# THUDM/GRAND-plus

Measured on AMD Instinct MI355X. Metric: propagation-matrix rows/sec (whole node), higher is better.
Workload: dtype f64

## Files before the change

grand_plus_amd/csrc/gfpush.hip:

```cpp
#include "gfpush_kernels.hpp"
#include "gfpush_sketch.hpp"
#ifndef GP_DIAG
#include "gfpush_dense.hpp"
#endif
#include "gfpush_plan.hpp"
#include "grandplus.h"

#include <dlfcn.h>
#include <sys/prctl.h>
#include <rccl/rccl.h>

#include <algorithm>
#include <atomic>
#include <cmath>
#include <cstdarg>
#include <cstdio>
#include <cstdlib>
#include <cstring>
#include <new>
#include <string>
#include <chrono>
#include <thread>
#include <type_traits>
#include <vector>
// ... 381 lines not shown

struct CallArgs {
    const int32_t* d_seeds; int64_t n_seeds; const double* coef; int n_coef; double rmax; int K;
    int32_t* d_row; int32_t* d_col; double* d_val; int32_t* d_filled; hipStream_t s;
};

struct CallShape : Shape {
    u64* timing_counters = nullptr;
    CallShape(const Shape& s, u64* tc = nullptr) : Shape(s), timing_counters(tc) {}
};

using Kernel = void (*)(KParams);
template <int... BLOCKS, class F> Kernel kernel_for(int block, F f) {
    Kernel k = nullptr;
    (void)(... || (block == BLOCKS && ((k = f(std::integral_constant<int, BLOCKS>())), true)));
    return k;
}

int resident_blocks(Kernel k, int block, int lds_bytes, int* out) {
    HIP_TRY(hipFuncSetAttribute(reinterpret_cast<const void*>(k), hipFuncAttributeMaxDynamicSharedMemorySize, lds_bytes));
    int nb = 0;
    HIP_TRY(hipOccupancyMaxActiveBlocksPerMultiprocessor(&nb, reinterpret_cast<const void*>(k), block, lds_bytes));
    *out = std::max(nb, 1);
    return GP_OK;
}
int launch_kernel(Kernel k, int block, const KParams& kp, int n_wg, int lds_bytes, hipStream_t s) {
    HIP_TRY(hipFuncSetAttribute(reinterpret_cast<const void*>(k), hipFuncAttributeMaxDynamicSharedMemorySize, lds_bytes));
    void* args[] = {const_cast<KParams*>(&kp)};
    (void)hipLaunchKernel(reinterpret_cast<const void*>(k), dim3(n_wg), dim3(block), args, lds_bytes, s);
    HIP_TRY(hipGetLastError());
    return GP_OK;
}

void use_slabs(KParams& kp, const Slabs& sl) {
    kp.push = sl.push; kp.push_cap = sl.push_cap;
    kp.bt = sl.bt; kp.bt_cap = sl.bt_cap;
    kp.resg = sl.resg; kp.resg_cap = sl.resg_cap;
    kp.log_key = sl.log_key; kp.log_val = sl.log_val; kp.log_cap = sl.log_cap;
    kp.log_pu = sl.log_pu; kp.arch = sl.arch; kp.arch_cap = sl.arch_cap;
    kp.cand = sl.cand; kp.cand_cap = sl.cand_cap;
    kp.bucket = sl.bucket; kp.bucket_cap = sl.bucket_cap;
}

void use_csr(KParams& kp, const gp_graph* g, bool acsr, bool general) {
    if (acsr) {
        kp.indices = g->d_acsr; kp.nnz = (int)(g->n_units << 5);
        kp.deg_shift = g->a_shift; kp.node_mask = g->a_mask; kp.deg_sat = g->a_sat;
        kp.node_pos = g->d_node_pos; kp.unit_info = g->d_unit_info; kp.sk_hub_units = g->a_sat > 32u ? 1u : 0u;
    } else {
        kp.indices = g->d_indices; kp.nnz = (int)g->nnz;
        kp.deg_shift = g->deg_shift; kp.node_mask = g->node_mask; kp.deg_sat = g->deg_sat;
    }
    kp.gk_acsr = acsr && general ? 1u : 0u;
}

int plan_status(Status st, const std::string& err) {
    return st == kOk ? GP_OK : fail(st == kNoMem ? GP_ERR_NOMEM : GP_ERR_INVALID_ARG, "%s", err.c_str());
}

#ifndef GP_DIAG
constexpr bool kDiagBuild = false;
Kernel sketch_kernel(int block) { return kernel_for<512, 1024, 768>(block, [](auto b) -> Kernel { return gfpush_sk_kernel<decltype(b)::value>; }); }

int plan_sketch(gp_graph* g, const CallArgs& a, const CallShape& shape, SketchPlan& p)
{
    sketch_wanted(kConsts, g->opt, g->est, shape, g->n_nodes, a.n_seeds, a.coef, a.n_coef, a.rmax, a.K, p);
    if (p.use) {
        int rc = ensure_acsr(g, a.s);
        if (rc) return rc;
        if (g->acsr_state != 1) p.use = false;
    }
    if (!p.use) return GP_OK;
    std::string err;
    int rc = plan_status(sketch_geometry(kConsts, g->opt, shape, a.K, p, err), err);
    if (rc || !p.use) return rc;
    int per_cu = 1;
    rc = resident_blocks(sketch_kernel(p.block), p.block, p.lds + g->opt.lds_pad, &per_cu);
    if (rc) return rc;
    p.wg = cap_workgroups(g->num_cus * per_cu, g->opt.max_workgroups, a.n_seeds);
    return GP_OK;
}

int launch_sketch(const gp_graph* g, KParams& kp, const CallArgs& a, const SketchPlan& sk, const u32* order)
{
    const Workspace& w = g->ws;
    use_slabs(kp, w.skl);
    kp.row_map = order; kp.n_rows_dev = nullptr; kp.queue_counter = kQueue;
    kp.retry_list = w.retry_list; kp.retry_counter = kRetryRows;
    kp.sk_lg_mu = sk.lg_mu; kp.sk_lg_mr = sk.lg_mr; kp.sk_cx = sk.cx;
    kp.sk_target = (u32)(g->opt.sk_target > 0 ? g->opt.sk_target : 4 * a.K);
    kp.sk_direct_max = g->opt.sk_direct_max > 0 ? (u32)g->opt.sk_direct_max : 0xFFFFFFFFu;
    kp.sk_rscale = 2147483648.0 / std::max(1.0, sk.coef_sum);
    {
        float t = (float)(a.rmax * 2147483648.0 * (1.0 - 1.0 / 1024.0));
        while ((double)t > a.rmax * 2147483648.0 * (1.0 - 1.0 / 1024.0)) t = std::nextafterf(t, 0.0f);
        kp.sk_thr_f = t;
    }
    use_csr(kp, g, true, false);
    return launch_kernel(sketch_kernel(sk.block), sk.block, kp, sk.wg, sk.lds + g->opt.lds_pad, a.s);
}
#else
constexpr bool kDiagBuild = true;
int plan_sketch(gp_graph*, const CallArgs&, const CallShape&, SketchPlan&) { return GP_OK; }
int launch_sketch(const gp_graph*, KParams&, const CallArgs&, const SketchPlan&, const u32*) { return GP_OK; }
#endif

Kernel general_kernel(int block) { return kernel_for<256, 512, 768, 1024>(block, [](auto b) -> Kernel { return gfpush_kernel<decltype(b)::value>; }); }
Kernel retry_kernel(int block) { return kernel_for<256, 512, 768, 1024>(block, [](auto b) -> Kernel { return gfpush_retry_kernel<decltype(b)::value>; }); }

int plan_general(gp_graph* g, const CallArgs& a, const CallShape& shape, SketchPlan& sk, GeneralPlan& p)
{
    CallInputs in;
    in.n_nodes = g->n_nodes; in.nnz = g->nnz; in.num_cus = g->num_cus;
    in.n_coef = a.n_coef; in.rmax = a.rmax; in.K = a.K; in.n_seeds = a.n_seeds;
    Occupancy occ;
    for (;;) {
        size_t free_b = 0, total_b = 0;
        const bool have_free = hipMemGetInfo(&free_b, &total_b) == hipSuccess;
        if (!have_free) (void)hipGetLastError();
        in.budget = workspace_budget(g->opt.workspace_mb, have_free, free_b, g->ws.bytes);
        Held held = g->ws.held();
        bool realloc = false; int need = 0; std::string err;
        Status st;
        while ((st = plan_general(kConsts, in, g->opt, shape, occ, sk, p, g->est, held, &realloc, &need, err)) == kNeedOccupancy) {
            int rc = resident_blocks(general_kernel(p.block_threads), p.block_threads, p.lds_bytes + g->opt.lds_pad, &occ.general[need]);
            if (rc) return rc;
        }
        if (st) return plan_status(st, err);
        if (!realloc) return GP_OK;
        int rc = allocate_workspace(g, held);
        if (rc == GP_ERR_NOMEM && sk.use && !shape.insists_on_sketch()) {
            sk.use = false; g_last_error.clear();
            continue;
        }
        return rc;
    }
}

KParams call_params(const gp_graph* g, const CallArgs& a, const GeneralPlan& gk, u64* counters)
{
    KParams kp;
    std::memset(&kp, 0, sizeof kp);
    kp.indptr = g->d_indptr; kp.indices = g->d_indices; kp.n_nodes = (int)g->n_nodes; kp.nnz = (int)g->nnz;
    kp.deg_shift = g->deg_shift; kp.node_mask = g->node_mask; kp.deg_sat = g->deg_sat;
    kp.seeds = a.d_seeds; kp.n_seeds = a.n_seeds;
    kp.coef = g->d_coef; kp.n_coef = a.n_coef; kp.rmax = a.rmax; kp.K = a.K;
    kp.out_row = a.d_row; kp.out_col = a.d_col; kp.out_val = a.d_val; kp.out_filled = a.d_filled;
    kp.counters = counters;
    kp.lds_slots = gk.lds_slots;
    kp.force_global = g->opt.force_global;
    kp.prune = prune_allowed(g->opt, a.coef, a.n_coef) ? 1 : 0;
    kp.diag_flags = g->opt.diag_flags;
    kp.rows_distinct = g->rows_distinct && g->opt.seedrow ? 1u : 0u;
    kp.solo = (g->opt.solo_levels ? 1u : 0u) | (g->opt.sk_seed_merge ? 2u : 0u);
    kp.direct = direct_tables(g->opt, g->n_nodes, gk) ? 1 : 0;
    return kp;
}

struct GeneralPass { const u32* rows; int n_rows; int queue; u32* overflow; int n_overflow; int overflow_queue; const u32* order; };

int launch_general(const gp_graph* g, KParams& kp, const GeneralPlan& gk, bool gk_acsr, const GeneralPass& pass, hipStream_t s)
{
    const Workspace& w = g->ws;
    const bool two_tier = w.big.n_wg > 0;
    use_csr(kp, g, gk_acsr, true);
    use_slabs(kp, w.est);
    kp.row_map = pass.rows ? pass.rows : pass.order; kp.n_rows_dev = pass.rows ? kp.counters + pass.n_rows : nullptr; kp.queue_counter = pass.queue;
    kp.retry_list = two_tier ? pass.overflow : nullptr; kp.retry_counter = pass.n_overflow;
    const Kernel k = pass.rows ? retry_kernel(gk.block_threads) : general_kernel(gk.block_threads);
    int rc = launch_kernel(k, gk.block_threads, kp, gk.n_wg, gk.lds_bytes + g->opt.lds_pad, s);
    if (rc || !two_tier) return rc;
    use_slabs(kp, w.big);
    kp.row_map = pass.overflow; kp.n_rows_dev = kp.counters + pass.n_overflow; kp.queue_counter = pass.overflow_queue;
    kp.retry_list = nullptr;
    return launch_kernel(retry_kernel(gk.block_threads), gk.block_threads, kp, w.big.n_wg, gk.lds_bytes + g->opt.lds_pad, s);
}

int enqueue_row_order(gp_graph* g, const CallArgs& a, bool acsr, hipStream_t s)
{
    const Workspace& w = g->ws;
    HIP_TRY(hipMemsetAsync(w.order_hist, 0, sizeof(uint32_t) * 64, s));
    const int shift = acsr ? g->a_shift : g->deg_shift;
    const u32 sat = acsr ? g->a_sat : g->deg_sat;
    const unsigned cost_wgs = (unsigned)std::min<int64_t>((a.n_seeds + 15) / 16, 4096), order_wgs = (unsigned)std::min<int64_t>((a.n_seeds + 255) / 256, 1024);
    hipLaunchKernelGGL(row_cost_kernel, dim3(cost_wgs), dim3(256), 0, s, a.d_seeds, (long long)a.n_seeds, (int)g->n_nodes, g->d_indptr,
                       acsr ? g->d_acsr : g->d_indices, acsr ? g->d_node_pos : (const u32*)nullptr, shift, sat, a.rmax, w.cost_cls, w.order_hist);
    hipLaunchKernelGGL(row_order_kernel, dim3(order_wgs), dim3(256), 0, s, w.cost_cls, (long long)a.n_seeds, w.order_hist, w.order_hist + 32, w.order);
    HIP_TRY(hipGetLastError());
    g->last_order_rows = a.n_seeds; g->last_order_sat = sat; g->last_order_shift = shift;
    return GP_OK;
}

int begin_call_state(gp_graph* g, const CallArgs& a, u64* counters, bool timing)
{
    const hipStream_t s = a.s;
    if (a.n_coef > g->coef_cap) {
        if (g->d_coef) (void)hipFree(g->d_coef);
        g->d_coef = nullptr; g->coef_cap = 0;
        HIP_TRY(hipMalloc(&g->d_coef, sizeof(double) * (size_t)a.n_coef));
        g->coef_cap = a.n_coef;
    }
    HIP_TRY(hipMemcpyAsync(g->d_coef, a.coef, sizeof(double) * (size_t)a.n_coef, hipMemcpyHostToDevice, s));
    if (timing || g->reset_pending) {
        HIP_TRY(hipMemsetAsync(counters, 0, sizeof(u64) * kNumCounters, s));
        if (!timing) { g->reset_pending = false; g->rows_total = 0; }
    } else {
        HIP_TRY(hipMemsetAsync(counters, 0, sizeof(u64) * (kSkSlabFails + 1), s));
        if (g->est.recipe_changed)
            HIP_TRY(hipMemsetAsync(counters + kMaxLevelEdges, 0, sizeof(u64) * 2, s));
    }
    g->est.recipe_changed = false;
    return GP_OK;
}

#ifndef GP_DIAG
static_assert(sizeof(DenseCtl) <= (size_t)kDenseCtlBytes, "DensePlan reserves kDenseCtlBytes for the dense kernel's control block");
Kernel dense_kernel(int block, bool staged) {
    return staged ? kernel_for<256, 512, 1024>(block, [](auto b) -> Kernel { return gfpush_dense_kernel<decltype(b)::value, true>; })
                  : kernel_for<256, 512, 1024>(block, [](auto b) -> Kernel { return gfpush_dense_kernel<decltype(b)::value, false>; });
}
bool dense_takes(const gp_graph* g, const CallArgs& a) {
    return dense_wanted(g->opt, g->n_nodes, g->nnz, a.n_coef, a.rmax, a.K, g->opt.lds_pad);
}

int enqueue_dense(gp_graph* g, const CallArgs& a, u64* counters, bool timing)
{
    const hipStream_t s = a.s;
    DensePlan dn = dense_plan(g->opt, g->n_nodes, g->nnz, a.K, g->opt.lds_pad);
    const Kernel k = dense_kernel(dn.block, dn.csr_lds);
    int per_cu = 1;
    int rc = resident_blocks(k, dn.block, dn.lds_bytes + g->opt.lds_pad, &per_cu);
    if (rc) return rc;
    dn = dense_plan(g->opt, g->n_nodes, g->nnz, a.K, g->opt.lds_pad, g->num_cus, per_cu, a.n_seeds);
    rc = ensure_packed(g, s);
    if (rc) return rc;
    rc = begin_call_state(g, a, counters, timing);
    if (rc) return rc;
    KParams kp = call_params(g, a, GeneralPlan(), counters);
    kp.direct = 0; kp.queue_counter = kQueue; kp.retry_counter = kRetryRows;
    kp.dn_hist = dn.off_hist; kp.dn_cur = dn.off_cur; kp.dn_next = dn.off_next; kp.dn_reserve = dn.off_reserve; kp.dn_marks = dn.off_marks;
    kp.dn_indptr = dn.off_indptr; kp.dn_indices = dn.off_indices; kp.dn_npad = (u32)dn.n_pad; kp.dn_csr_lds = dn.csr_lds ? 1u : 0u;
    HIP_TRY(hipEventRecord(g->ev0, s));
    g->last_order_rows = 0;
    if (a.n_seeds > 0) {
        rc = launch_kernel(k, dn.block, kp, dn.workgroups, dn.lds_bytes + g->opt.lds_pad, s);
        if (rc) return rc;
    }
    HIP_TRY(hipEventRecord(g->ev1, s));
    HIP_TRY(hipMemcpyAsync(g->h_counters, counters, sizeof(u64) * kNumCounters, hipMemcpyDeviceToHost, s));
    g->last_stream = s; g->est.last_call_rows = a.n_seeds; g->est.grown_for_call = false;
    g->est.last_kind = 3; g->est.last_sk_soft = false;
    if (timing) return GP_OK;
    g->launched = true;
    std::memset(&g->last, 0, sizeof g->last);
    g->rows_total += a.n_seeds;
    g->last.rows = g->rows_total;
    g->last.kernel = 3;
    g->last.workgroups = dn.workgroups; g->last.block_threads = dn.block; g->last.lds_bytes = dn.lds_bytes;
    return GP_OK;
}
#else
bool dense_takes(const gp_graph*, const CallArgs&) { return false; }
int enqueue_dense(gp_graph*, const CallArgs&, u64*, bool) { return GP_OK; }
#endif

int enqueue_call(gp_graph* g, const CallArgs& a, const CallShape& shape)
{
    const hipStream_t s = a.s;
    const bool timing = shape.timing_counters != nullptr;
    u64* const counters = timing ? shape.timing_counters : g->d_counters;
    if (g->launched && g->last_stream != s) HIP_TRY(hipStreamSynchronize(g->last_stream));
    if (!g->est.grown_for_call && g->est.rmax == a.rmax && g->est.n_coef == a.n_coef) {
        const hipError_t qs = hipStreamQuery(g->last_stream);
        if (qs == hipSuccess) grow_estimate(g);
        else if (qs != hipErrorNotReady) (void)hipGetLastError();
    }

    if (dense_takes(g, a)) return enqueue_dense(g, a, counters, timing);

    SketchPlan sk; GeneralPlan gk;
    int rc = plan_sketch(g, a, shape, sk);
    if (rc) return rc;
    rc = plan_general(g, a, shape, sk, gk);
    if (rc) return rc;
    rc = ensure_packed(g, s);
    if (rc) return rc;
    Workspace& w = g->ws;

    rc = begin_call_state(g, a, counters, timing);
    if (rc) return rc;
    if (w.dirty) {
        hipLaunchKernelGGL(init_tables_kernel, dim3(4096), dim3(256), 0, s, w.est.resg, (u64)w.est.n_wg * w.est.resg_cap);
        if (w.big.n_wg > 0)
            hipLaunchKernelGGL(init_tables_kernel, dim3(1024), dim3(256), 0, s, w.big.resg, (u64)w.big.n_wg * w.big.resg_cap);
        HIP_TRY(hipGetLastError());
        w.dirty = false;
    }

    KParams kp = call_params(g, a, gk, counters);
    bool gk_acsr = general_wants_acsr(kDiagBuild, g->opt, kp.direct != 0, g->n_nodes, a.n_seeds);
    if (gk_acsr) { rc = ensure_acsr(g, s); if (rc) return rc; gk_acsr = g->acsr_state == 1; }

    HIP_TRY(hipEventRecord(g->ev0, s));
    const u32* order = nullptr;
    g->last_order_rows = 0;
    if (g->opt.row_order && a.n_seeds > (sk.use ? sk.wg : gk.n_wg) && a.n_seeds <= w.retry_cap && a.n_seeds <= (int64_t)0xFFFFFFFFll) {
        rc = enqueue_row_order(g, a, sk.use || gk_acsr, s);
// ... 189 lines not shown
int gp_graph_create(const int32_t* indptr, int64_t n_nodes, const int32_t* indices, int64_t nnz,
                    int device, gp_graph** out)
{
    g_last_error.clear();
    if (!out) return fail(GP_ERR_NULL, "out is NULL");
    *out = nullptr;
    if (!indptr || (!indices && nnz > 0)) return fail(GP_ERR_NULL, "indptr/indices is NULL");
    if (n_nodes < 0 || nnz < 0 || n_nodes >= 2147483647ll || nnz >= 2147483647ll)
        return fail(GP_ERR_INVALID_CSR, "n_nodes=%lld nnz=%lld outside int32 CSR range", (long long)n_nodes, (long long)nnz);
    if (indptr[0] != 0) return fail(GP_ERR_INVALID_CSR, "indptr[0] = %d, expected 0", indptr[0]);
    for (int64_t i = 0; i < n_nodes; ++i)
        if (indptr[i + 1] < indptr[i]) return fail(GP_ERR_INVALID_CSR, "indptr decreases at node %lld", (long long)i);
    if (indptr[n_nodes] != nnz) return fail(GP_ERR_INVALID_CSR, "indptr[n] = %d but nnz = %lld", indptr[n_nodes], (long long)nnz);
    using clk = std::chrono::steady_clock;
    auto ms_since = [](clk::time_point t) { return std::chrono::duration<double, std::milli>(clk::now() - t).count(); };
    clk::time_point t0 = clk::now();
    const int ndev = gp_device_count();
    if (ndev <= 0) return fail(GP_ERR_NO_DEVICE, "no HIP device is visible (this library has no CPU path)");
    if (device < 0 || device >= ndev) return fail(GP_ERR_NO_DEVICE, "device %d outside [0, %d)", device, ndev);
    HIP_TRY(hipSetDevice(device));
    hipDeviceProp_t prop;
    HIP_TRY(hipGetDeviceProperties(&prop, device));
    g_create_ms[0] = ms_since(t0); t0 = clk::now();

    gp_graph* g = new (std::nothrow) gp_graph();
    if (!g) return fail(GP_ERR_NOMEM, "host allocation failed");
    g->device = device; g->n_nodes = n_nodes; g->nnz = nnz;
    g->num_cus = prop.multiProcessorCount;
    auto cleanup = [&](int status) { gp_graph_destroy(g); return status; };
    u32* d_flags = nullptr;
    {
        const size_t b_idx = (sizeof(int) * (size_t)(nnz + 1) + 255) & ~(size_t)255, b_ptr = (sizeof(int) * (size_t)(n_nodes + 1) + 255) & ~(size_t)255;
        if (hipMalloc(&g->d_csr_block, b_idx + b_ptr + 256) != hipSuccess)
            return cleanup(fail(GP_ERR_NOMEM, "hipMalloc of the CSR (%lld nodes, %lld nnz) failed", (long long)n_nodes, (long long)nnz));
        g->d_indices = (int*)g->d_csr_block; g->d_indptr = (int*)((char*)g->d_csr_block + b_idx); d_flags = (u32*)((char*)g->d_csr_block + b_idx + b_ptr);
    }
    if (hipStreamCreateWithFlags(&g->stream, hipStreamNonBlocking) != hipSuccess)
        return cleanup(fail(GP_ERR_HIP, "creating per-graph HIP objects failed"));
    g_create_ms[1] = ms_since(t0); t0 = clk::now();
    Stager stager;
    if (stager.copy(g->d_indptr, indptr, sizeof(int) * (size_t)(n_nodes + 1), g->stream) != GP_OK ||
        (nnz > 0 && stager.copy(g->d_indices, indices, sizeof(int) * (size_t)nnz, g->stream) != GP_OK) ||
        hipMemsetAsync(g->d_indices + nnz, 0xFF, sizeof(int), g->stream) != hipSuccess ||
        hipMemsetAsync(d_flags, 0, sizeof(u32) * 2, g->stream) != hipSuccess)
        return cleanup(fail(GP_ERR_HIP, "CSR upload failed"));
    g_create_ms[2] = ms_since(t0); t0 = clk::now();
    u32 h_flags[2] = {0u, 0u};
    if (n_nodes > 0) hipLaunchKernelGGL(csr_check_kernel, dim3(8192), dim3(256), 0, g->stream, g->d_indptr, g->d_indices, (long long)n_nodes, d_flags);
    if (hipGetLastError() != hipSuccess ||
        hipMemcpyAsync(h_flags, d_flags, sizeof h_flags, hipMemcpyDeviceToHost, g->stream) != hipSuccess ||
        hipStreamSynchronize(g->stream) != hipSuccess)
        return cleanup(fail(GP_ERR_HIP, "CSR validation on the device failed"));
    if (h_flags[0]) return cleanup(fail(GP_ERR_INVALID_CSR, "a column id is outside [0, %lld)", (long long)n_nodes));
    g->rows_distinct = h_flags[1] == 0;
    g_create_ms[3] = ms_since(t0); t0 = clk::now();
    if (hipMalloc(&g->d_counters, sizeof(u64) * kNumCounters) != hipSuccess ||
        hipHostMalloc(&g->h_counters, sizeof(u64) * kNumCounters) != hipSuccess ||
        hipEventCreate(&g->ev0) != hipSuccess || hipEventCreate(&g->ev1) != hipSuccess)
        return cleanup(fail(GP_ERR_HIP, "creating per-graph HIP objects failed"));
    g_create_ms[4] = ms_since(t0);
    *out = g;
    return GP_OK;
}

void gp_graph_destroy(gp_graph* g) {
    if (!g) return;
    if (g->multi) {
        for (size_t d = 0; d < g->comms.size(); ++d) if (g->comms[d]) (void)g_rccl.CommDestroy(g->comms[d]);
        for (size_t d = 0; d < g->part.size(); ++d) {
            if (!g->part[d]) continue;
            (void)hipSetDevice(g->devices[d]);
            if (d < g->m_slab.size() && g->m_slab[d]) (void)hipFree(g->m_slab[d]);
            if (d < g->m_gather.size() && g->m_gather[d]) (void)hipFree(g->m_gather[d]);
            if (d < g->m_seeds.size() && g->m_seeds[d]) (void)hipFree(g->m_seeds[d]);
            gp_graph_destroy(g->part[d]);
        }
        if (g->m_host) (void)hipHostFree(g->m_host);
        delete g;
        return;
    }
    (void)hipSetDevice(g->device);
    if (g->launched) (void)hipStreamSynchronize(g->last_stream);
    free_workspace(g->ws);
    if (g->d_csr_block) (void)hipFree(g->d_csr_block);
    else {
        if (g->d_indptr) (void)hipFree(g->d_indptr);
        if (g->d_indices) (void)hipFree(g->d_indices);
    }
    if (g->d_acsr) (void)hipFree(g->d_acsr);
    if (g->d_node_pos) (void)hipFree(g->d_node_pos);
    if (g->d_unit_info) (void)hipFree(g->d_unit_info);
    if (g->d_counters) (void)hipFree(g->d_counters);
    if (g->d_cal_counters) (void)hipFree(g->d_cal_counters);
    if (g->d_wg_log) (void)hipFree(g->d_wg_log);
    if (g->h_counters) (void)hipHostFree(g->h_counters);
    if (g->d_coef) (void)hipFree(g->d_coef);
    if (g->d_seeds) (void)hipFree(g->d_seeds);
    for (int i = 0; i < 2; ++i) if (g->h_slab[i]) (void)hipHostFree(g->h_slab[i]);
    if (g->ev0) (void)hipEventDestroy(g->ev0);
    if (g->ev1) (void)hipEventDestroy(g->ev1);
    if (g->stream) (void)hipStreamDestroy(g->stream);
    delete g;
}

int64_t gp_graph_num_nodes(const gp_graph* g) { return g ? g->n_nodes : -1; }
int64_t gp_graph_nnz(const gp_graph* g) { return g ? g->nnz : -1; }
int gp_graph_device(const gp_graph* g) { return g ? (g->multi ? g->devices[0] : g->device) : -1; }
int gp_graph_num_gpus(const gp_graph* g) { return g ? (g->multi ? g->n_parts : 1) : -1; }

int gp_set_option(gp_graph* g, const char* key, int64_t value) {
    if (!g || !key) return fail(GP_ERR_NULL, "null argument");
    const std::string k(key);
    if (g->multi) {
        if (k == "force_collective") { g->force_collective = value ? 1 : 0; return GP_OK; }
        if (k == "gather_host") {
            if (!value && g->shared_devices) return fail(GP_ERR_INVALID_ARG, "parts of this handle share a device: RCCL takes one rank per device, the gather stays on the host");
            g->gather_host = value ? 1 : 0; return GP_OK;
        }
        if (k == "min_rows_per_gpu") {
            if (value < 1) return fail(GP_ERR_INVALID_ARG, "min_rows_per_gpu must be >= 1");
            g->min_rows_per_gpu = value; return GP_OK;
        }
        for (gp_graph* q : g->part) if (q) { int rc = gp_set_option(q, key, value); if (rc) return rc; }
        return GP_OK;
    }
    if (k == "block_threads") {
        if (value != 256 && value != 512 && value != 768 && value != 1024) return fail(GP_ERR_INVALID_ARG, "block_threads must be 256, 512, 768 or 1024");
        g->opt.block_threads = (int)value;
    } else if (k == "lds_bytes") {
        if (value < 40 * 1024 || value > 160 * 1024) return fail(GP_ERR_INVALID_ARG, "lds_bytes must be in [40960, 163840]");
        g->opt.lds_bytes = (int)(value & ~15ll);
    } else if (k == "lds_pad") {
        if (value < 0 || value > 120 * 1024) return fail(GP_ERR_INVALID_ARG, "lds_pad must be in [0, 122880]");
        g->opt.lds_pad = (int)(value & ~15ll);
    } else if (k == "kernel") {
        if (value < 0 || value > 3) return fail(GP_ERR_INVALID_ARG, "kernel must be 0 (automatic), 1 (general), 2 (sketch) or 3 (dense)");
        g->opt.kernel = (int)value;
    } else if (k == "dn_block_threads") {
        if (value != 0 && value != 256 && value != 512 && value != 1024) return fail(GP_ERR_INVALID_ARG, "dn_block_threads must be 0, 256, 512 or 1024");
        g->opt.dn_block = (int)value;
    } else if (k == "dn_csr_lds") {
        g->opt.dn_csr_lds = value ? 1 : 0;
    } else if (k == "sk_block_threads") {
        if (value != 0 && value != 512 && value != 768 && value != 1024) return fail(GP_ERR_INVALID_ARG, "sk_block_threads must be 0, 512, 768 or 1024");
        g->opt.sk_block = (int)value;
    } else if (k == "sk_lg_mu" || k == "sk_lg_mr") {
        if (value != 0 && (value < 8 || value > 14)) return fail(GP_ERR_INVALID_ARG, "%s must be 0 or in [8, 14]", key);
        (k == "sk_lg_mu" ? g->opt.sk_lg_mu : g->opt.sk_lg_mr) = (int)value;
    } else if (k == "sk_direct_max") {
        if (value < 0 || value > (1 << 20)) return fail(GP_ERR_INVALID_ARG, "sk_direct_max must be in [0, 2^20]");
        g->opt.sk_direct_max = (int)value;
    } else if (k == "sk_seed_merge") {
        g->opt.sk_seed_merge = value ? 1 : 0;
    } else if (k == "row_order") {
        g->opt.row_order = value ? 1 : 0;
    } else if (k == "gk_acsr") {
        g->opt.gk_acsr = value ? 1 : 0;
    } else if (k == "sk_target") {
        if (value < 0 || value > 4096) return fail(GP_ERR_INVALID_ARG, "sk_target must be in [0, 4096]");
        g->opt.sk_target = (int)value;
    } else if (k == "measure_choice") {
        g->opt.measure_choice = value ? 1 : 0;
        if (!value) g->choices.clear();
    } else if (k == "verify_merge") {
        g->opt.verify_merge = value ? 1 : 0;
    } else if (k == "pretouch") {
        g->opt.pretouch = value ? 1 : 0;
    } else if (k == "max_workgroups") {
        if (value < 0 || value > 65535) return fail(GP_ERR_INVALID_ARG, "max_workgroups must be in [0, 65535]");
        g->opt.max_workgroups = (int)value;
    } else if (k == "workspace_mb") {
        if (value < 1) return fail(GP_ERR_INVALID_ARG, "workspace_mb must be >= 1");
        g->opt.workspace_mb = value;
    } else if (k == "est_level_edges") {
        if (value < 0) return fail(GP_ERR_INVALID_ARG, "est_level_edges must be >= 0");
        g->opt.est_level_edges = value;
    } else if (k == "force_global") {
        g->opt.force_global = value ? 1 : 0;
    } else if (k == "exact_stats") {
        g->opt.exact_stats = value ? 1 : 0;
    } else if (k == "direct_tables") {
        g->opt.direct_tables = value ? 1 : 0;
    } else if (k == "solo_levels") {
        g->opt.solo_levels = value ? 1 : 0;
    } else if (k == "seedrow") {
        g->opt.seedrow = value ? 1 : 0;
    } else if (k == "diag_flags") {
        g->opt.diag_flags = (int)value;
    } else if (k == "max_degree_bits") {
        if (g->packed) return fail(GP_ERR_INVALID_ARG, "max_degree_bits must be set before the first gfpush call");
        if (value < 0 || value > 31) return fail(GP_ERR_INVALID_ARG, "max_degree_bits must be in [0, 31]");
        g->opt.max_degree_bits = (int)value;
    } else {
        return fail(GP_ERR_INVALID_ARG, "unknown option '%s'", key);
    }
    if (k == "max_workgroups" || k == "workspace_mb" || k == "lds_pad" || k == "est_level_edges" || k.rfind("sk_", 0) == 0 || k.rfind("dn_", 0) == 0 ||
        k == "solo_levels" || k == "seedrow" || k == "direct_tables") g->choices.clear();
    return GP_OK;
}

int gp_gfpush_device(gp_graph* g, const int32_t* d_seeds, int64_t n_seeds,
                     const double* coef, int n_coef, double rmax, int K,
                     int32_t* d_row, int32_t* d_col, double* d_val, int32_t* d_filled, void* stream)
{
    g_last_error.clear();
    int rc = check_call_args(g, n_seeds, coef, n_coef, rmax, K);
    if (rc) return rc;
    if (g->multi) return fail(GP_ERR_INVALID_ARG, "gp_gfpush_device needs a single-GPU graph (device buffers live on one GPU); "
                                                  "a multi-GPU handle takes host buffers through gp_gfpush");
    if (n_seeds > 0 && (!d_seeds || !d_row || !d_col || !d_val)) return fail(GP_ERR_NULL, "a device buffer is NULL");
    HIP_TRY(hipSetDevice(g->device));
    const CallArgs a{d_seeds, n_seeds, coef, n_coef, rmax, K, d_row, d_col, d_val, d_filled, (hipStream_t)stream};
    const gp_graph::Choice* c = nullptr;
    rc = measured_choice(g, a, &c);
    if (rc) return rc;
    CallShape shape(Shape{g->opt.kernel, g->opt.block_threads, g->opt.lds_bytes, false});
    if (c) shape = CallShape(Shape{c->kernel, c->block_threads, c->lds_bytes, true});
    if (c) std::memcpy(g->last_cal_ms, c->ms, sizeof g->last_cal_ms);
    else std::memset(g->last_cal_ms, 0, sizeof g->last_cal_ms);
    return enqueue_call(g, a, shape);
}

int gp_reset_stats(gp_graph* g) {
    if (!g) return fail(GP_ERR_NULL, "graph handle is NULL");
    if (g->multi) { for (gp_graph* q : g->part) if (q) (void)gp_reset_stats(q); g->m_has_stats = false; return GP_OK; }
    g->reset_pending = true;
    return GP_OK;
}

int gp_get_stats(gp_graph* g, gp_stats* out) {
    if (!g) return fail(GP_ERR_NULL, "graph handle is NULL");
    if (g->multi) {
        if (out) { if (g->m_has_stats) *out = g->m_last; else std::memset(out, 0, sizeof *out); }
        if (g->m_has_stats && g->m_last.failed_rows)
            return fail(GP_ERR_OVERFLOW, "%lld row(s) hit a workspace bound", (long long)g->m_last.failed_rows);
        return GP_OK;
    }
    if (!g->launched) { if (out) std::memset(out, 0, sizeof *out); return GP_OK; }
    HIP_TRY(hipSetDevice(g->device));
    HIP_TRY(hipStreamSynchronize(g->last_stream));
    float ms = 0.f;
    HIP_TRY(hipEventElapsedTime(&ms, g->ev0, g->ev1));
    gp_stats& s = g->last;
    s.kernel_ms = ms;
    s.pushes = (int64_t)g->h_counters[kPushes];
    s.edges = (int64_t)g->h_counters[kEdges];
    s.filled = (int64_t)g->h_counters[kFilled];
    s.support = (int64_t)g->h_counters[kSupport];
    s.frontier = (int64_t)g->h_counters[kFrontier];
    s.lds_levels = (int64_t)g->h_counters[kLdsLevels];
    s.global_levels = (int64_t)g->h_counters[kGlobalLevels];
    s.failed_rows = (int64_t)g->h_counters[kFailedRows];
    s.degree_lookups = (int64_t)g->h_counters[kDegLookups];
    s.retried_rows = (int64_t)g->h_counters[kRetriedTotal];
    s.max_level_edges = (int64_t)g->h_counters[kMaxLevelEdges];
    s.max_log_records = (int64_t)g->h_counters[kMaxLogRecords];
    s.sketch_candidate_edges = (int64_t)g->h_counters[kSkCandEdges];
    s.sketch_second_sweeps = (int64_t)g->h_counters[kSkSweep2];
    for (int i = 0; i < 3; ++i) s.choice_ms[i] = g->last_cal_ms[i];
    grow_estimate(g);
    s.diag_ticks_scan = (int64_t)g->h_counters[kTicksScan];
    s.diag_ticks_expand = (int64_t)g->h_counters[kTicksExpand];
    s.diag_ticks_topk = (int64_t)g->h_counters[kTicksTopk];
    s.diag_ticks_total = (int64_t)g->h_counters[kTicksTotal];
    s.diag_ticks_scan_hbm = (int64_t)g->h_counters[kTicksScanHbm];
    s.diag_ticks_expand_hbm = (int64_t)g->h_counters[kTicksExpandHbm];
    for (int i = 0; i < 16; ++i) s.diag_sub[i] = (int64_t)g->h_counters[kDiag0 + i];
    if (out) *out = s;
    if (s.failed_rows) {
        g->ws.dirty = true;
        return fail(GP_ERR_OVERFLOW, "%lld row(s) hit a workspace bound or had an out-of-range seed", (long long)s.failed_rows);
    }
    return GP_OK;
}

int gp_gfpush(gp_graph* g, const int32_t* seeds, int64_t n_seeds,
              const double* coef, int n_coef, double rmax, int K,
              int32_t* row_idx, int32_t* col_idx, double* value)
{
    g_last_error.clear();
    int rc = check_call_args(g, n_seeds, coef, n_coef, rmax, K);
    if (rc) return rc;
    if (n_seeds == 0) return GP_OK;
    if (!seeds || !row_idx || !col_idx || !value) return fail(GP_ERR_NULL, "a host buffer is NULL");
    for (int64_t i = 0; i < n_seeds; ++i)
        if (seeds[i] < 0 || seeds[i] >= g->n_nodes)
            return fail(GP_ERR_INVALID_SEED, "node_idx[%lld] = %d outside [0, %lld)", (long long)i, seeds[i], (long long)g->n_nodes);
    if (g->multi) return gfpush_multi(g, seeds, n_seeds, coef, n_coef, rmax, K, row_idx, col_idx, value);
    HIP_TRY(hipSetDevice(g->device));
    if (n_seeds > g->seeds_cap) {
        if (g->d_seeds) (void)hipFree(g->d_seeds);
        g->d_seeds = nullptr; g->seeds_cap = 0;
        HIP_TRY(hipMalloc(&g->d_seeds, sizeof(int) * (size_t)n_seeds));
        g->seeds_cap = n_seeds;
    }
    const PackedSlab lay(n_seeds, K);
    const size_t need_bytes = lay.bytes;
    if (need_bytes > g->out_bytes) {
        for (int i = 0; i < 2; ++i) { if (g->h_slab[i]) (void)hipHostFree(g->h_slab[i]); g->h_slab[i] = nullptr; g->h_slab_clean[i] = false; }
        g->out_bytes = 0;
        for (int i = 0; i < 2; ++i) HIP_TRY(hipHostMalloc(&g->h_slab[i], need_bytes, hipHostMallocMapped | hipHostMallocCoherent));
        g->out_bytes = need_bytes;
    }
    const int cur = g->h_slab_next; g->h_slab_next ^= 1;
    char* hb = g->h_slab[cur];
    if (!g->h_slab_clean[cur]) std::memset(hb, 0xFF, g->out_bytes);
    g->h_slab_clean[cur] = false;
    char* idle = g->h_slab[cur ^ 1]; size_t idle_done = g->h_slab_clean[cur ^ 1] ? g->out_bytes : 0;
    double* d_val = nullptr; int* d_row = nullptr; int* d_col = nullptr; int* d_filled = nullptr;
    {
        void* dp = nullptr;
        HIP_TRY(hipHostGetDevicePointer(&dp, hb, 0));
        d_val = (double*)((char*)dp + lay.val); d_row = (int*)((char*)dp + lay.row); d_col = (int*)((char*)dp + lay.col); d_filled = (int*)((char*)dp + lay.filled);
    }
    hipStream_t s = g->stream;
    g->reset_pending = true;
    HIP_TRY(hipMemcpyAsync(g->d_seeds, seeds, sizeof(int) * (size_t)n_seeds, hipMemcpyHostToDevice, s));
    rc = gp_gfpush_device(g, g->d_seeds, n_seeds, coef, n_coef, rmax, K, d_row, d_col, d_val, d_filled, s);
    if (rc) return rc;
    MergeState merge;
    std::vector<unsigned char>& done = g->h_done;
    done.assign((size_t)n_seeds, 0);
    auto sweep = [&]() { merge_sweep(hb, lay, K, n_seeds, done.data(), merge, row_idx, col_idx, value); };
    struct Resetter {
        std::thread t;
        ~Resetter() { if (t.joinable()) t.join(); }
    } resetter;
    bool reset_inline = false;
    if (idle_done < g->out_bytes) {
        const size_t n_reset = g->out_bytes;
        try { resetter.t = std::thread([idle, n_reset]() { std::memset(idle, 0xFF, n_reset); }); }
        catch (...) { reset_inline = true; }
    }
    struct TimerSlack {
        long old = -1;
        TimerSlack() { old = prctl(PR_GET_TIMERSLACK, 0, 0, 0, 0); if (old > 0) (void)prctl(PR_SET_TIMERSLACK, 1000UL, 0, 0, 0); }
        ~TimerSlack() { if (old > 0) (void)prctl(PR_SET_TIMERSLACK, (unsigned long)old, 0, 0, 0); }
    } timer_slack;
    for (;;) {
        const hipError_t q = hipStreamQuery(s);
        if (q == hipSuccess) break;
        if (q != hipErrorNotReady) { (void)hipGetLastError(); break; }
        const int64_t before = merge.n_merged;
        sweep();
        if (merge.n_merged - before < 256) std::this_thread::sleep_for(std::chrono::microseconds(60));
    }
    if (resetter.t.joinable()) { resetter.t.join(); g->h_slab_clean[cur ^ 1] = true; }
    else if (reset_inline) { std::memset(idle, 0xFF, g->out_bytes); g->h_slab_clean[cur ^ 1] = true; }
    rc = gp_get_stats(g, nullptr);
    if (rc) return rc;
    for (int spin = 0; merge.n_merged != n_seeds && spin < 2000000; ++spin) sweep();
    if (merge.n_merged != n_seeds) return fail(GP_ERR_HIP, "%lld of %lld rows never arrived in host memory", (long long)(n_seeds - merge.n_merged), (long long)n_seeds);
    if (g->opt.verify_merge) {
        int64_t first_bad = -1;
        const int64_t bad = verify_merged(hb, lay, K, n_seeds, row_idx, col_idx, value, &first_bad);
        if (bad) return fail(GP_ERR_HIP, "verify_merge: %lld of %lld rows were merged before they had fully arrived (first: row %lld)",
                             (long long)bad, (long long)n_seeds, (long long)first_bad);
    }
    return GP_OK;
}

int gp_graph_create_multi_on(const int32_t* indptr, int64_t n_nodes, const int32_t* indices, int64_t nnz,
                             const int* devices, int n_parts, gp_graph** out)
{
    g_last_error.clear();
    if (!out) return fail(GP_ERR_NULL, "out is NULL");
    *out = nullptr;
    if (!devices || n_parts < 1) return fail(GP_ERR_INVALID_ARG, "gp_graph_create_multi_on needs at least one device");
    const int ndev = gp_device_count();
    if (ndev <= 0) return fail(GP_ERR_NO_DEVICE, "no HIP device is visible (this library has no CPU path)");
    bool repeated = false;
    for (int d = 0; d < n_parts; ++d) {
        if (devices[d] < 0 || devices[d] >= ndev) return fail(GP_ERR_NO_DEVICE, "device %d outside [0, %d)", devices[d], ndev);
        for (int e = 0; e < d; ++e) repeated |= devices[e] == devices[d];
    }
    gp_graph* first = nullptr;
    int rc = gp_graph_create(indptr, n_nodes, indices, nnz, devices[0], &first);
    if (rc) return rc;
    gp_graph* g = new (std::nothrow) gp_graph();
    if (!g) { gp_graph_destroy(first); return fail(GP_ERR_NOMEM, "host allocation failed"); }
    g->multi = true; g->n_parts = n_parts; g->n_nodes = n_nodes; g->nnz = nnz;
    g->part.assign(n_parts, nullptr); g->devices.assign(devices, devices + n_parts);
    g->part[0] = first;
    g->comms.assign(n_parts, nullptr);
    g->m_slab.assign(n_parts, nullptr); g->m_gather.assign(n_parts, nullptr); g->m_seeds.assign(n_parts, nullptr);
    g->shared_devices = repeated;
    if (repeated) g->gather_host = 1;
    *out = g;
    return GP_OK;
}

int gp_graph_create_multi(const int32_t* indptr, int64_t n_nodes, const int32_t* indices, int64_t nnz,
                          int n_gpus, gp_graph** out)
{
    g_last_error.clear();
    if (!out) return fail(GP_ERR_NULL, "out is NULL");
    *out = nullptr;
    const int ndev = gp_device_count();
    if (ndev <= 0) return fail(GP_ERR_NO_DEVICE, "no HIP device is visible (this library has no CPU path)");
    if (n_gpus < 0 || n_gpus > ndev) return fail(GP_ERR_NO_DEVICE, "n_gpus = %d but %d device(s) are visible", n_gpus, ndev);
    if (n_gpus == 0) n_gpus = ndev;
    std::vector<int> devs(n_gpus);
    for (int d = 0; d < n_gpus; ++d) devs[d] = d;
    return gp_graph_create_multi_on(indptr, n_nodes, indices, nnz, devs.data(), n_gpus, out);
}

}

namespace {

int replicate_part(gp_graph* g, int d) {
    gp_graph* src = g->part[0];
    HIP_TRY(hipSetDevice(src->device));
    int rc = ensure_packed(src, src->stream);
    if (rc) return rc;
    HIP_TRY(hipStreamSynchronize(src->stream));
    const int dev = g->devices[d];
    HIP_TRY(hipSetDevice(dev));
    hipDeviceProp_t prop;
    HIP_TRY(hipGetDeviceProperties(&prop, dev));
    gp_graph* q = new (std::nothrow) gp_graph();
    if (!q) return fail(GP_ERR_NOMEM, "host allocation failed");
    struct Guard { gp_graph* q; ~Guard() { if (q) gp_graph_destroy(q); } } guard{q};
    q->device = dev; q->n_nodes = src->n_nodes; q->nnz = src->nnz; q->num_cus = prop.multiProcessorCount;
    q->deg_shift = src->deg_shift; q->node_mask = src->node_mask; q->deg_sat = src->deg_sat;
    q->packed = true; q->opt.max_degree_bits = src->opt.max_degree_bits; q->rows_distinct = src->rows_distinct;
    q->opt.block_threads = src->opt.block_threads; q->opt.lds_bytes = src->opt.lds_bytes; q->opt.max_workgroups = src->opt.max_workgroups;
    q->opt.workspace_mb = src->opt.workspace_mb; q->opt.force_global = src->opt.force_global; q->opt.exact_stats = src->opt.exact_stats;
    q->opt.direct_tables = src->opt.direct_tables; q->opt.est_level_edges = src->opt.est_level_edges; q->opt.seedrow = src->opt.seedrow; q->opt.solo_levels = src->opt.solo_levels;
    q->opt.kernel = src->opt.kernel; q->opt.row_order = src->opt.row_order; q->opt.gk_acsr = src->opt.gk_acsr; q->opt.sk_seed_merge = src->opt.sk_seed_merge; q->opt.sk_block = src->opt.sk_block; q->opt.sk_lg_mu = src->opt.sk_lg_mu; q->opt.sk_lg_mr = src->opt.sk_lg_mr; q->opt.sk_target = src->opt.sk_target; q->opt.lds_pad = src->opt.lds_pad; q->opt.sk_direct_max = src->opt.sk_direct_max;
    const size_t b_ptr = sizeof(int) * (size_t)(q->n_nodes + 1), b_idx = sizeof(int) * (size_t)(q->nnz + 1);
    HIP_TRY(hipMalloc(&q->d_indptr, b_ptr));
    HIP_TRY(hipMalloc(&q->d_indices, b_idx));
    if (dev == src->device) {
        HIP_TRY(hipMemcpy(q->d_indptr, src->d_indptr, b_ptr, hipMemcpyDeviceToDevice));
        HIP_TRY(hipMemcpy(q->d_indices, src->d_indices, b_idx, hipMemcpyDeviceToDevice));
    } else {
        HIP_TRY(hipMemcpyPeer(q->d_indptr, dev, src->d_indptr, src->device, b_ptr));
        HIP_TRY(hipMemcpyPeer(q->d_indices, dev, src->d_indices, src->device, b_idx));
    }
    HIP_TRY(hipMalloc(&q->d_counters, sizeof(u64) * kNumCounters));
    HIP_TRY(hipHostMalloc(&q->h_counters, sizeof(u64) * kNumCounters));
    HIP_TRY(hipEventCreate(&q->ev0));
    HIP_TRY(hipEventCreate(&q->ev1));
    HIP_TRY(hipStreamCreateWithFlags(&q->stream, hipStreamNonBlocking));
    guard.q = nullptr;
    g->part[d] = q;
    return GP_OK;
}

int gfpush_multi(gp_graph* g, const int32_t* seeds, int64_t n_seeds, const double* coef, int n_coef, double rmax, int K,
                 int32_t* row_idx, int32_t* col_idx, double* value)
{
    const MultiPlan plan = plan_multi(n_seeds, K, g->n_parts, g->min_rows_per_gpu, g->force_collective != 0, g->gather_host != 0);
    const int G = plan.G, Gc = plan.Gc;
    if (plan.single) {
        int rc = gp_gfpush(g->part[0], seeds, n_seeds, coef, n_coef, rmax, K, row_idx, col_idx, value);
        gp_stats st; const int rc2 = gp_get_stats(g->part[0], &st);
        g->m_last = st; g->m_has_stats = true;
        return rc ? rc : rc2;
    }
    const bool collective = !g->gather_host;
    for (int d = 1; d < Gc; ++d)
        if (!g->part[d]) { int rc = replicate_part(g, d); if (rc) return rc; }
    if (collective && !g->comms_ready) {
        int rc = load_rccl();
        if (rc) return rc;
        RCCL_TRY(g_rccl.CommInitAll(g->comms.data(), g->n_parts, g->devices.data()));
        g->comms_ready = true;
    }
    const int64_t per = plan.per;
    const size_t stride = plan.stride;
    if (g->m_cap_stride.size() != (size_t)g->n_parts) { g->m_cap_stride.assign(g->n_parts, 0); g->m_cap_per.assign(g->n_parts, 0); }
    for (int d = 0; d < Gc; ++d) {
        if (g->m_slab[d] && g->m_cap_stride[d] >= stride && g->m_cap_per[d] >= per) continue;
        HIP_TRY(hipSetDevice(g->devices[d]));
        if (g->m_slab[d]) (void)hipFree(g->m_slab[d]);
        if (g->m_gather[d]) (void)hipFree(g->m_gather[d]);
        if (g->m_seeds[d]) (void)hipFree(g->m_seeds[d]);
        g->m_slab[d] = g->m_gather[d] = nullptr; g->m_seeds[d] = nullptr; g->m_cap_stride[d] = 0; g->m_cap_per[d] = 0;
        const size_t cap_s = std::max(stride, g->m_cap_stride[d]);
        const int64_t cap_p = std::max<int64_t>(std::max(per, g->m_cap_per[d]), 1);
        HIP_TRY(hipMalloc(&g->m_slab[d], cap_s));
        HIP_TRY(hipMalloc(&g->m_gather[d], cap_s * (size_t)g->n_parts));
        HIP_TRY(hipMalloc(&g->m_seeds[d], sizeof(int) * (size_t)cap_p));
        g->m_cap_stride[d] = cap_s; g->m_cap_per[d] = cap_p;
    }
    if (stride * (size_t)g->n_parts > g->m_host_bytes) {
        if (g->m_host) (void)hipHostFree(g->m_host);
        g->m_host = nullptr; g->m_host_bytes = 0;
        HIP_TRY(hipSetDevice(g->devices[0]));
        HIP_TRY(hipHostMalloc(&g->m_host, stride * (size_t)g->n_parts));
        g->m_host_bytes = stride * (size_t)g->n_parts;
    }
    const size_t cur_stride = stride;
    const int64_t cur_per = per;
    const PackedSlab lay(cur_per, K);

    std::vector<int> rcs(Gc, GP_OK);
    std::vector<std::string> errs(Gc);
    std::vector<std::thread> pool;
    auto work = [&](int d) {
        gp_graph* q = g->part[d];
        int64_t lo, n;
        plan_block(plan, d, n_seeds, &lo, &n);
        auto run = [&]() -> int {
            HIP_TRY(hipSetDevice(q->device));
            char* slab = g->m_slab[d];
            HIP_TRY(hipMemsetAsync(slab + lay.filled, 0, 4 * (size_t)cur_per, q->stream));
            if (n > 0) {
                HIP_TRY(hipMemcpyAsync(g->m_seeds[d], seeds + lo, sizeof(int) * (size_t)n, hipMemcpyHostToDevice, q->stream));
                q->reset_pending = true;
                int rc = gp_gfpush_device(q, g->m_seeds[d], n, coef, n_coef, rmax, K, (int*)(slab + lay.row),
                                          (int*)(slab + lay.col), (double*)(slab + lay.val), (int*)(slab + lay.filled), q->stream);
                if (rc) return rc;
            }
            if (!collective) HIP_TRY(hipMemcpyAsync(g->m_host + (size_t)d * cur_stride, slab, cur_stride, hipMemcpyDeviceToHost, q->stream));
            return GP_OK;
        };
        rcs[d] = run();
        if (rcs[d]) errs[d] = g_last_error;
    };
    for (int d = 1; d < Gc; ++d) pool.emplace_back(work, d);
    work(0);
    for (auto& th : pool) th.join();
    for (int d = 0; d < Gc; ++d) if (rcs[d]) { g_last_error = errs[d]; return rcs[d]; }

    if (collective) {
        RCCL_TRY(g_rccl.GroupStart());
        for (int d = 0; d < Gc; ++d)
            RCCL_TRY(g_rccl.AllGather(g->m_slab[d], g->m_gather[d], cur_stride, ncclUint8, g->comms[d], g->part[d]->stream));
        RCCL_TRY(g_rccl.GroupEnd());
        HIP_TRY(hipSetDevice(g->devices[0]));
        HIP_TRY(hipMemcpyAsync(g->m_host, g->m_gather[0], cur_stride * (size_t)Gc, hipMemcpyDeviceToHost, g->part[0]->stream));
    }
    gp_stats sum; std::memset(&sum, 0, sizeof sum);
    int status = GP_OK;
    for (int d = 0; d < Gc; ++d) {
        gp_graph* q = g->part[d];
        HIP_TRY(hipSetDevice(q->device));
        HIP_TRY(hipStreamSynchronize(q->stream));
        int64_t lo_d, n_d;
        plan_block(plan, d, n_seeds, &lo_d, &n_d);
        if (!q->launched || n_d == 0) continue;
        gp_stats st; const int rc = gp_get_stats(q, &st);
        if (rc && !status) status = rc;
        sum.rows += st.rows; sum.pushes += st.pushes; sum.edges += st.edges; sum.filled += st.filled; sum.support += st.support;
        sum.frontier += st.frontier; sum.lds_levels += st.lds_levels; sum.global_levels += st.global_levels;
        sum.failed_rows += st.failed_rows; sum.degree_lookups += st.degree_lookups; sum.retried_rows += st.retried_rows;
        sum.kernel_ms = std::max(sum.kernel_ms, st.kernel_ms); sum.workgroups += st.workgroups;
        sum.block_threads = st.block_threads; sum.lds_bytes = st.lds_bytes; sum.lds_slots = st.lds_slots;
        sum.workspace_bytes += st.workspace_bytes;
        sum.max_level_edges = std::max(sum.max_level_edges, st.max_level_edges);
        sum.max_log_records = std::max(sum.max_log_records, st.max_log_records);
    }
    g->m_last = sum; g->m_has_stats = true;
    if (status) return status;
    for (int d = 0; d < G; ++d) {
        int64_t lo, n;
        plan_block(plan, d, n_seeds, &lo, &n);
        scatter_filled(g->m_host + (size_t)d * cur_stride, cur_per, K, lo, n, row_idx, col_idx, value);
    }
    return GP_OK;
}

}
```

grand_plus_amd/csrc/gfpush_kernels.hpp:

```cpp
#pragma once

#include <hip/hip_runtime.h>
#include <stdint.h>

#include "gfpush_hash.hpp"

namespace gp {

typedef unsigned long long u64;
typedef unsigned int u32;

#define GP_LDS  __attribute__((address_space(3)))
#define GP_KARG __attribute__((address_space(4)))
template <class T> __device__ __forceinline__ T* lds_at(u32 byte_off) { return (T*)(GP_LDS T*)(uintptr_t)byte_off; }
__device__ __forceinline__ u32 uni(u32 x) { return (u32)__builtin_amdgcn_readfirstlane((int)x); }
__device__ __forceinline__ int uni(int x) { return __builtin_amdgcn_readfirstlane(x); }
__device__ __forceinline__ u64 uni(u64 x) { return ((u64)uni((u32)(x >> 32)) << 32) | uni((u32)x); }
__device__ __forceinline__ long long uni(long long x) { return (long long)uni((u64)x); }
__device__ __forceinline__ double uni(double x) {
    const u64 b = (u64)__double_as_longlong(x);
    return __longlong_as_double((long long)(((u64)uni((u32)(b >> 32)) << 32) | uni((u32)b)));
}

constexpr int    kEmpty      = -1;
constexpr int    kCoefLds    = 40;
constexpr u32    kUnitShift  = 6;
constexpr int    kTopkBins   = 4096;
constexpr int    kBucketCap  = 256;
#ifndef GP_FLAT_W
#define GP_FLAT_W 4
#endif
constexpr int    kFlatW      = GP_FLAT_W;
#if defined(GP_DIAG) && !defined(GP_DIAG_LIGHT)
#define GP_DIAG_HEAVY 1
#endif
#ifdef GP_DIAG
constexpr int    kCtlStruct  = 4096;
#elif defined(GP_SK_TIMING)
constexpr int    kCtlStruct  = 2048;
#else
constexpr int    kCtlStruct  = 1280;
#endif
constexpr int    kCtlBytes   = kCtlStruct + 16 * 64 * kFlatW;
constexpr int    kThreeLds   = 53248;
#ifndef GP_TOPK_UF
#define GP_TOPK_UF 12
#endif
#ifndef GP_MIN_CAP
#define GP_MIN_CAP 1024
#endif
#ifndef GP_CAP_MULT
#define GP_CAP_MULT 4
#endif
#ifndef GP_SCAN_VC
#define GP_SCAN_VC 2
#endif
constexpr u32    kMinCap     = GP_MIN_CAP;
constexpr u32    kMaxParts   = 64;
#ifndef GP_LOAD_NUM
#define GP_LOAD_NUM 3u
#define GP_LOAD_DEN 4u
#endif
#ifndef GP_BUCKET_MIN
#define GP_BUCKET_MIN 4
#endif
constexpr u32    kBucketMin  = GP_BUCKET_MIN;
constexpr u32    kSkUnitShift = 5;
constexpr u32    kSkMaxPushers = 65536;

struct PushEntry { u32 rel; u32 off; double share; };
struct ResRec    { int key;   int pad; double val; };
struct Cand      { u64 bits;  int key; int pad;  };

struct LevelCtr {
    double dangling;
    u32 n_dangling;
    u32 n_rec;
    u64 alloc;
    u64 pad1;
};

struct Ctl {
    long long row;
    LevelCtr lc[2];
    u32 bcnt[64];
    u32 boff[65];
    u32 log_count;
    u32 n_cand;
    u32 ovf;
    u32 fail;
    u32 n_sel;
    u32 n_bucket;
    u32 tk_bin;
    u32 tk_above;
    u32 tk_count;
    u32 bovf;
    u64 st[12];
    u32 tk_wide;
    u64 st_row[12];
    double coef[kCoefLds];
    double thr_early;
    double tau_early;
    u32 n_heavy;
    u32 heavy_from;
    u32 heavy_ovf;
    u32 pad_heavy;
    u32 ratio_q[16];
#ifdef GP_DIAG
    u64 lvl_acc[16][6];
    u64 row_acc[4];
    u64 barw[16];
    u32 barn[16];
    u64 exp_c0, exp_c2, exp_pre, exp_post;
    u32 exp_max, exp_pad; u64 exp_sum_max, exp_sum_all;
    u64 exp_sub[8];
    u64 scan_sub[4];
    u64 site_w[64];
    u32 site_n[64];
#endif
};
static_assert(sizeof(Ctl) <= (size_t)kCtlStruct, "the control block must fit its LDS reservation");
enum Stat { sPush = 0, sEdges, sFront, sDeg, sFilled, sSupport, sLds, sGlb, sFailed, sNumStats };
__device__ __forceinline__ void stat_add(Ctl* ctl, int which, u64 n) {
    __hip_atomic_fetch_add(&ctl->st_row[which], n, __ATOMIC_RELAXED, __HIP_MEMORY_SCOPE_WORKGROUP);
}
__device__ __forceinline__ void stat_add_final(Ctl* ctl, int which, u64 n) {
    __hip_atomic_fetch_add(&ctl->st[which], n, __ATOMIC_RELAXED, __HIP_MEMORY_SCOPE_WORKGROUP);
}
__device__ __forceinline__ u32 wave_incl_scan_dpp(u32 x) {
    x += (u32)__builtin_amdgcn_update_dpp(0, (int)x, 0x111, 0xF, 0xF, false);
    x += (u32)__builtin_amdgcn_update_dpp(0, (int)x, 0x112, 0xF, 0xF, false);
    x += (u32)__builtin_amdgcn_update_dpp(0, (int)x, 0x114, 0xF, 0xF, false);
    x += (u32)__builtin_amdgcn_update_dpp(0, (int)x, 0x118, 0xF, 0xF, false);
    x += (u32)__builtin_amdgcn_update_dpp(0, (int)x, 0x142, 0xA, 0xF, false);
    x += (u32)__builtin_amdgcn_update_dpp(0, (int)x, 0x143, 0xC, 0xF, false);
    return x;
}
__device__ __forceinline__ u32 wave_id() { return (u32)__builtin_amdgcn_readfirstlane((int)(threadIdx.x >> 6)); }
__device__ __forceinline__ u32 wave_sum32(u32 x) {
    return (u32)__builtin_amdgcn_readlane((int)wave_incl_scan_dpp(x), 63);
}

enum Counter { kQueue = 0, kQueueRetry, kRetryRows,
               kQueueRetry2, kRetryRows2,
               kSkSlabFails,
               kMaxLevelEdges, kMaxLogRecords,
               kRetriedTotal,
               kPushes, kEdges, kFilled, kSupport, kFrontier, kLdsLevels,
               kGlobalLevels, kFailedRows, kDegLookups,
               kSkCandEdges, kSkSweep2,
               kTicksScan, kTicksExpand, kTicksTopk, kTicksTotal, kTicksScanHbm, kTicksExpandHbm,
               kDiag0, kDiagLast = kDiag0 + 15,
               kDiagX0, kDiagXLast = kDiagX0 + 255,
               kNumCounters };

enum OvfCount { kOvfLevel = 8,
                kOvfSolo = 9,
                kOvfTopk = 10 };
#if !defined(GP_DIAG) && !defined(GP_SK_TIMING)
#define GP_OVF_COUNT(p, which) __hip_atomic_fetch_add(&(p).counters[kDiag0 + (which)], 1ull, __ATOMIC_RELAXED, __HIP_MEMORY_SCOPE_AGENT)
#else
#define GP_OVF_COUNT(p, which) do { } while (0)
#endif

#ifdef GP_DIAG_HEAVY
constexpr int kSyncBase = __COUNTER__;
#define GP_SYNC() do { constexpr int site_ = (__COUNTER__ - kSyncBase - 1) & 63; const u64 tb_ = clock64(); __syncthreads(); if ((threadIdx.x & 63) == 0) { const u64 w_ = clock64() - tb_; ctl->barw[threadIdx.x >> 6] += w_; ++ctl->barn[threadIdx.x >> 6]; \
    __hip_atomic_fetch_add(&ctl->site_w[site_], w_, __ATOMIC_RELAXED, __HIP_MEMORY_SCOPE_WORKGROUP); __hip_atomic_fetch_add(&ctl->site_n[site_], 1u, __ATOMIC_RELAXED, __HIP_MEMORY_SCOPE_WORKGROUP); } } while (0)
#else
#define GP_SYNC() __syncthreads()
#endif
#ifdef GP_DIAG
#define GP_STAMP(var) do { if (threadIdx.x == 0) var = wall_clock64(); } while (0)
#define GP_ACCUM(acc, t0, t1) do { if (threadIdx.x == 0) acc += (t1) - (t0); } while (0)
#define GP_SUB_BEGIN() do { if (threadIdx.x == 0) gp_sub_t = wall_clock64(); } while (0)
#define GP_SUB(i) do { if (threadIdx.x == 0) { const u64 n_ = wall_clock64(); gp_sub_acc[i] += n_ - gp_sub_t; gp_sub_t = n_; } } while (0)
#define GP_SUB_COUNT(i, n) do { if (threadIdx.x == 0) gp_sub_acc[i] += (n); } while (0)
#else
#define GP_STAMP(var) do { } while (0)
#define GP_ACCUM(acc, t0, t1) do { } while (0)
#define GP_SUB_BEGIN() do { } while (0)
#define GP_SUB(i) do { } while (0)
#define GP_SUB_COUNT(i, n) do { } while (0)
#endif
#ifdef GP_DIAG
#define GP_SUB_PARAMS , u64& gp_sub_t, u64 (&gp_sub_acc)[16]
#define GP_SUB_ARGS , gp_sub_t, gp_sub_acc
#else
#define GP_SUB_PARAMS
#define GP_SUB_ARGS
#endif

struct KParams {
    const int* indptr; const int* indices; int n_nodes;
    int nnz;
    int deg_shift; u32 node_mask; u32 deg_sat;
    const int* seeds; long long n_seeds;
    const double* coef; int n_coef; double rmax; int K;
    int* out_row; int* out_col; double* out_val; int* out_filled;
    PushEntry* push; u64 push_cap;
    u32* bt; u64 bt_cap;
    ResRec* resg;    u64 resg_cap;
    int* log_key; double* log_val; u64 log_cap;
    Cand* cand;      u64 cand_cap;
    ResRec* bucket;  u64 bucket_cap;
    u64* counters;
    u32 lds_slots;
    int force_global;
    int prune;
    u32 solo;
    u32 rows_distinct;
    int direct;
    const u32* row_map; const u64* n_rows_dev; u32* retry_list; int queue_counter;
    int retry_counter; int pad_rc;
    u32 sk_lg_mu, sk_lg_mr, sk_cx, sk_target; float sk_thr_f; u32 sk_direct_max; double sk_rscale;
    const u32* node_pos;
    const int* unit_info;
    unsigned short* log_pu; double* arch; u64 arch_cap;
    u32 sk_hub_units; u32 gk_acsr;
    int diag_flags;
    int pad_df;
    u64* wg_log;
    u32 dn_hist, dn_cur, dn_next, dn_reserve, dn_marks, dn_indptr, dn_indices, dn_npad, dn_csr_lds, dn_pad;
};
typedef const GP_KARG KParams& KP;
static_assert(sizeof(KParams) % 8 == 0, "kparams(): the hidden kernel arguments must start right behind KParams");
__device__ __forceinline__ KP kparams() {
    return *(const GP_KARG KParams*)((const GP_KARG char*)__builtin_amdgcn_implicitarg_ptr() - sizeof(KParams));
}

__device__ __forceinline__ void csr_row(KP p, u32 key, int& ds, int& de) {
    const u32 id = key & p.node_mask;
    if (p.gk_acsr) {
        u32 deg = key >> p.deg_shift;
        if (deg == p.deg_sat) {
            if (p.sk_hub_units) deg = (u32)p.unit_info[id + 1u];
            else { const int node = p.unit_info[id]; deg = (u32)(p.indptr[node + 1] - p.indptr[node]); }
        }
        ds = (int)(id << kSkUnitShift); de = ds + (int)deg;
    } else { ds = p.indptr[id]; de = p.indptr[id + 1]; }
}

static_assert(kMinCap > 2 * kProbeSpan, "every LDS table must be much larger than the probe span");

template <class T> __device__ __forceinline__ T ld_l2(const T* p) {
    return __hip_atomic_load(p, __ATOMIC_RELAXED, __HIP_MEMORY_SCOPE_AGENT);
}
template <class T> __device__ __forceinline__ void st_l2(T* p, T v) {
    __hip_atomic_store(p, v, __ATOMIC_RELAXED, __HIP_MEMORY_SCOPE_AGENT);
}

__device__ __forceinline__ u32 wave_incl_scan(u32 x, int ) { return wave_incl_scan_dpp(x); }
__device__ __forceinline__ u32 wave_suffix_scan(u32 x, int lane) {
#pragma unroll
    for (int d = 1; d < 64; d <<= 1) {
        const u32 y = __shfl_down(x, d);
        if (lane + d < 64) x += y;
    }
    return x;
}
__device__ __forceinline__ u64 wave_sum64(u64 x) {
#pragma unroll
    for (int d = 32; d >= 1; d >>= 1) x += __shfl_down(x, d);
    return __shfl(x, 0);
}

__device__ __forceinline__ u32 wave_alloc(u32* lds_counter, u32 n, int lane) {
    const u32 incl = wave_incl_scan(n, lane);
    const u32 total = __shfl(incl, 63);
    u32 base = 0;
    if (total != 0) {
        if (lane == 63)
            base = __hip_atomic_fetch_add(lds_counter, total, __ATOMIC_RELAXED, __HIP_MEMORY_SCOPE_WORKGROUP);
        base = __shfl(base, 63);
    }
    return base + incl - n;
}

__device__ __forceinline__ u32 lane_prefix(u64 mask) {
    return __builtin_amdgcn_mbcnt_hi((u32)(mask >> 32), __builtin_amdgcn_mbcnt_lo((u32)mask, 0u));
}
__device__ __forceinline__ u32 wave_alloc1(u32* lds_counter, bool flag, int lane) {
    const u64 m = __ballot(flag);
    if (m == 0) return 0;
    u32 base = 0;
    if (lane == 0)
        base = __hip_atomic_fetch_add(lds_counter, (u32)__popcll(m), __ATOMIC_RELAXED, __HIP_MEMORY_SCOPE_WORKGROUP);
    base = (u32)__builtin_amdgcn_readfirstlane((int)base);
    return base + lane_prefix(m);
}
template <int U>
__device__ __forceinline__ void wave_alloc_flags(u32* lds_counter, const bool (&flag)[U], u32 (&idx)[U], int lane) {
    u64 m[U]; u32 total = 0;
#pragma unroll
    for (int u = 0; u < U; ++u) { m[u] = __ballot(flag[u]); total += (u32)__popcll(m[u]); }
#pragma unroll
    for (int u = 0; u < U; ++u) idx[u] = 0;
    if (total == 0) return;
    u32 base = 0;
    if (lane == 0)
        base = __hip_atomic_fetch_add(lds_counter, total, __ATOMIC_RELAXED, __HIP_MEMORY_SCOPE_WORKGROUP);
    base = (u32)__builtin_amdgcn_readfirstlane((int)base);
#pragma unroll
    for (int u = 0; u < U; ++u) { idx[u] = base + lane_prefix(m[u]); base += (u32)__popcll(m[u]); }
}

__device__ __forceinline__ u32 lds_addr(const void* p) {
    return (u32)(uintptr_t)(const __attribute__((address_space(3))) void*)p;
}
__device__ __forceinline__ int probe_cas_asm(int* keys, u32& slot, int k) {
    int seen; u32 ad; u64 sv; u32 st;
    asm volatile(
        "s_mov_b64 %[sv], exec\n\t"
        "s_mov_b32 %[st], 1\n"
        "1:\n\t"
        "v_lshl_add_u32 %[ad], %[sl], 2, %[base]\n\t"
// ... 1999 lines not shown
```

grand_plus_amd/csrc/gfpush_plan.hpp:

```cpp
#pragma once

#include <algorithm>
#include <atomic>
#include <cmath>
#include <cstddef>
#include <cstdint>
#include <cstdio>
#include <cstring>
#include <string>

namespace gp {
namespace planning {

typedef unsigned long long cap_t;

enum Status { kOk = 0, kInvalidArg, kNoMem, kNeedOccupancy };

struct KernelConsts {
    int ctl_bytes = 0, three_lds = 0, min_cap = 0, topk_bins = 0, bucket_cap = 0, unit_shift = 0;
    int sk_max_pushers = 0, sk_max_coef = 0, sk_tie = 0;
};

struct Options {
    int block_threads = 0; int lds_bytes = 0; int max_workgroups = 0;
    int verify_merge = 0;
    int lds_pad = 0; int pretouch = 0;
    int64_t workspace_mb = 65536; int force_global = 0; int exact_stats = 0; int diag_flags = 0; int direct_tables = 1; int seedrow = 1; int solo_levels = 1;
    int kernel = 0;
    int sk_block = 0, sk_lg_mu = 0, sk_lg_mr = 0, sk_target = 0, sk_direct_max = 0;
    int row_order = 1;
    int sk_seed_merge = 1; int gk_acsr = 1;
    int64_t est_level_edges = 0;
    int measure_choice = 1;
    int max_degree_bits = 31;
    int dn_block = 0; int dn_csr_lds = 0;
};

struct Estimate {
    int kind = 0; int last_kind = 1;
    bool sk_auto_off = false; double sk_off_rmax = 0.0; int sk_off_n_coef = 0;
    bool last_sk_soft = false;
    double edges = 0.0, log = 0.0;
    double rmax = -1.0; int n_coef = 0;
    bool recipe_changed = false;
    double cur_edges = 0.0, cur_log = 0.0;
    int64_t last_call_rows = 0; bool grown_for_call = true;
};


struct SlabCaps {
    int n_wg = 0;
    cap_t push_cap = 0, resg_cap = 0, log_cap = 0, cand_cap = 0, bucket_cap = 0, bt_cap = 0;
    cap_t arch_cap = 0;
    size_t log_bytes() const { return arch_cap ? 6 * (size_t)log_cap + 8 * (size_t)arch_cap : 12 * (size_t)log_cap; }
    size_t per_wg() const { return 16 * (size_t)(2 * push_cap + resg_cap + cand_cap + bucket_cap) + log_bytes() + 8 * (size_t)bt_cap + 64; }
    bool covers(const SlabCaps& o) const {
        if (o.n_wg == 0) return true;
        return n_wg >= o.n_wg && push_cap >= o.push_cap && resg_cap >= o.resg_cap && log_cap >= o.log_cap &&
               cand_cap >= o.cand_cap && bucket_cap >= o.bucket_cap && bt_cap >= o.bt_cap && arch_cap >= o.arch_cap && (arch_cap != 0) == (o.arch_cap != 0);
    }
    void widen(const SlabCaps& o) {
        if (o.n_wg == 0 || (n_wg != 0 && (arch_cap != 0) != (o.arch_cap != 0))) return;
        n_wg = std::max(n_wg, o.n_wg); push_cap = std::max(push_cap, o.push_cap); resg_cap = std::max(resg_cap, o.resg_cap);
        log_cap = std::max(log_cap, o.log_cap); cand_cap = std::max(cand_cap, o.cand_cap); bucket_cap = std::max(bucket_cap, o.bucket_cap);
        bt_cap = std::max(bt_cap, o.bt_cap); arch_cap = std::max(arch_cap, o.arch_cap);
    }
};

struct SlabOffsets {
    static constexpr size_t kAbsent = ~(size_t)0;
    size_t push = 0, resg = 0, cand = 0, bucket = 0, arch = kAbsent, log_val = kAbsent, log_key = 0, bt = 0, log_pu = kAbsent, bytes = 0;
};
inline SlabOffsets carve_offsets(const SlabCaps& c, int wgs) {
    SlabOffsets o;
    size_t q = 0;
    o.push = q;    q += 16 * (size_t)wgs * 2 * c.push_cap;
    o.resg = q;    q += 16 * (size_t)wgs * c.resg_cap;
    o.cand = q;    q += 16 * (size_t)wgs * c.cand_cap;
    o.bucket = q;  q += 16 * (size_t)wgs * c.bucket_cap;
    if (c.arch_cap) { o.arch = q; q += 8 * (size_t)wgs * c.arch_cap; }
    else            { o.log_val = q; q += 8 * (size_t)wgs * c.log_cap; }
    o.log_key = q; q += 4 * (size_t)wgs * c.log_cap;
    o.bt = q;      q += 4 * (size_t)wgs * 2 * c.bt_cap;
    if (c.arch_cap) { o.log_pu = q; q += 2 * (size_t)wgs * c.log_cap; }
    o.bytes = (q + 255) & ~(size_t)255;
    return o;
}

inline double level_edge_bound_of(int64_t nnz) { return (double)nnz + 16.0; }

inline SlabCaps slab_sizes(const KernelConsts& kc, int64_t n_nodes, int64_t nnz, int n_coef, double e_max, double log_records) {
    const double n_d = (double)n_nodes;
    const double f_max = std::min(n_d, e_max) + 1.0;
    const double L = (double)(n_coef - 1);
    double logn = (L + 1.0) * f_max + 64.0;
    if (log_records > 0.0) logn = std::min(logn, log_records + 64.0);
    const double supp = std::max(1.0, std::min(std::min(n_d, 1.0 + L * f_max), logn));
    SlabCaps sl;
    sl.resg_cap = (cap_t)std::max(2048.0, 2.0 * f_max);
    sl.log_cap = ((cap_t)logn + 3) & ~3ull;
    sl.cand_cap = (cap_t)supp + 1;
    sl.push_cap = (cap_t)(f_max + 2.0);
    const double e_bt = std::min(level_edge_bound_of(nnz), std::max(8.0 * e_max, 1048576.0));
    sl.bt_cap = (((cap_t)std::max(e_max, e_bt) >> kc.unit_shift) + 4) & ~1ull;
    sl.bucket_cap = (cap_t)e_max + 2;
    return sl;
}

inline SlabCaps sk_slab_sizes(const KernelConsts& kc, int64_t n_nodes, int64_t nnz, double e_max, double log_records, bool at_bound) {
    SlabCaps sl;
    sl.log_cap = ((cap_t)std::min(log_records + 64.0, 4.0e9) + 3) & ~3ull;
    sl.push_cap = (cap_t)(std::min((double)n_nodes, at_bound ? e_max : std::max(e_max / 4.0, 4096.0)) + 2.0);
    const double e_bt = std::min(level_edge_bound_of(nnz), std::max(8.0 * e_max, 1048576.0));
    sl.bt_cap = (((cap_t)std::max(e_max, e_bt) >> kc.unit_shift) + 4) & ~1ull;
    sl.arch_cap = (cap_t)std::min((double)kc.sk_max_pushers, std::max(at_bound ? (double)sl.log_cap : (double)sl.log_cap / 4.0, 4096.0));
    sl.arch_cap = (sl.arch_cap + 3) & ~3ull;
    return sl;
}

inline double level_edge_bound(int64_t nnz, double rmax) {
    double e = (double)nnz;
    if (rmax > 0.0) e = std::min(e, std::floor(1.001 / rmax) + 16.0);
    return e;
}


struct Held { bool have = false; SlabCaps est, skl, big; int64_t retry_cap = 0; size_t bytes = 0; };

struct WorkspacePlan {
    SlabCaps est, skl, big;
    bool fits = false;
    int64_t retry_cap = 0; size_t total = 0;
};

inline size_t workspace_budget(int64_t workspace_mb, bool have_free, size_t free_bytes, size_t held_bytes) {
    size_t budget = (size_t)workspace_mb << 20;
    if (have_free) budget = std::min(budget, (size_t)(0.9 * (double)(free_bytes + held_bytes)));
    return budget;
}

inline Status plan_workspace(const KernelConsts& kc, int64_t n_nodes, int64_t nnz, int n_coef, double rmax, int n_wg, int sk_wg,
                             int64_t n_seeds, size_t budget, int64_t est_level_edges, Estimate& e, const Held& held,
                             WorkspacePlan& out, std::string& err) {
    const double bound = level_edge_bound(nnz, rmax);
    {
        const SlabCaps worst = slab_sizes(kc, n_nodes, nnz, n_coef, bound, 0.0);
        if (2.0 * (double)worst.resg_cap > 8.0e9 || (double)worst.log_cap > 4.0e9) {
            char buf[160];
            std::snprintf(buf, sizeof buf, "workspace bound exceeds 32-bit record space (order %d, rmax %g)", n_coef - 1, rmax);
            err = buf;
            return kInvalidArg;
        }
    }
    const int kind = sk_wg > 0 ? 2 : 1;
    if (e.rmax != rmax || e.n_coef != n_coef || e.kind != kind) {
        e.rmax = rmax; e.n_coef = n_coef; e.kind = kind; e.edges = 0.0; e.log = 0.0;
        e.recipe_changed = true;
    }
    double e_est = est_level_edges > 0 ? (double)est_level_edges
                                       : std::max(e.edges, std::max(32768.0, bound / 4.0));
    e_est = std::min(e_est, bound);
    double log_est = e_est >= bound ? 0.0 : std::max(e.log, 4.0 * e_est);
    SlabCaps est, skl;
    auto plan = [&]() {
        est = slab_sizes(kc, n_nodes, nnz, n_coef, e_est, log_est);
        if (sk_wg > 0) skl = sk_slab_sizes(kc, n_nodes, nnz, e_est, log_est > 0.0 ? log_est : (double)n_coef * e_est, !(log_est > 0.0));
        return (double)est.per_wg() * n_wg + (sk_wg > 0 ? (double)skl.per_wg() * sk_wg : 0.0);
    };
    while (plan() > 0.5 * (double)budget && e_est > 4096.0) {
        e_est *= 0.75; log_est = std::max(4096.0, 0.75 * (log_est > 0.0 ? log_est : (double)est.log_cap));
    }
    if (plan() > 0.5 * (double)budget) {
        if (sk_wg > 0) { err = "workspace_mb too small for the sketch kernel's slabs"; return kNoMem; }
        n_wg = (int)std::max<size_t>(1, budget / 2 / est.per_wg());
    }
    e.cur_edges = e_est; e.cur_log = log_est;
    est.n_wg = n_wg; skl.n_wg = sk_wg;
    SlabCaps big;
    if (e_est < bound || log_est > 0.0) {
        big = slab_sizes(kc, n_nodes, nnz, n_coef, bound, 0.0);
        const size_t used = est.per_wg() * (size_t)n_wg + skl.per_wg() * (size_t)sk_wg;
        const size_t left = budget - std::min(budget, used);
        int nb = (int)std::min<size_t>(8, left / std::max<size_t>(1, big.per_wg()));
        if (nb < 1) {
// ... 353 lines not shown
```

grand_plus_amd/csrc/gfpush_sketch.hpp:

```cpp
#pragma once

#include "gfpush_kernels.hpp"

#ifndef GP_DIAG

namespace gp {

#ifndef GP_SK_SWEEP_DEPTH
#define GP_SK_SWEEP_DEPTH 2
#endif
constexpr int kSkMaxCoef = 40;
constexpr u32 kSkTie     = 256;

struct CtlS {
    long long row;
    LevelCtr lc[2];
    u32 ovf;
    u32 fail;
    u32 n_sel, n_tie;
    u32 tk_bin, tk_above, tk_count, tk_total;
    u32 tk_t, tk_wide, tk_dig;
    u64 kth_bits;
    u32 bcnt[64];
    u64 st[8], st_row[8];
    double coef[kSkMaxCoef + 1];
    u32 cand_q[kSkMaxCoef];
    int seed_key; u32 tot_pu, tot_log;
    double lv_dang; u32 lv_has_dang;
    u32 max_e, max_log;
    u32 k_log_cap, k_pu_cap, k_direct_max, k_solo_ok, k_cx, k_pad; double k_rscale;
#ifdef GP_SK_TIMING
    u64 tacc[16]; u64 tlast;
    u64 tacc2[14]; u64 tlast2;
    u64 t_enter, t_row, row_sum, row_max;
    u64 row_hist[32];
#endif
};
#ifdef GP_SK_TIMING
#define SKT_BEGIN(ctl) do { if (threadIdx.x == 0) (ctl)->tlast = wall_clock64(); } while (0)
#define SKT(ctl, i) do { if (threadIdx.x == 0) { const u64 n_ = wall_clock64(); (ctl)->tacc[i] += n_ - (ctl)->tlast; (ctl)->tlast = n_; } } while (0)
#define SKT_COUNT(ctl, i, n) do { if (threadIdx.x == 0) (ctl)->tacc[i] += (n); } while (0)
#define SKT2_BEGIN(ctl) do { if (threadIdx.x == 0) (ctl)->tlast2 = wall_clock64(); } while (0)
#define SKT2(ctl, i) do { if (threadIdx.x == 0) { const u64 n_ = wall_clock64(); (ctl)->tacc2[i] += n_ - (ctl)->tlast2; (ctl)->tlast2 = n_; } } while (0)
#else
#define SKT_BEGIN(ctl) do { } while (0)
#define SKT(ctl, i) do { } while (0)
#define SKT_COUNT(ctl, i, n) do { } while (0)
#define SKT2_BEGIN(ctl) do { } while (0)
#define SKT2(ctl, i) do { } while (0)
#endif
static_assert(sizeof(CtlS) <= (size_t)kCtlStruct, "the control block must fit its LDS reservation");
enum StatS { zPush = 0, zEdges, zDeg, zFilled, zLevels, zFailed, zCand, zSweep2, zNumStats };
__device__ __forceinline__ void zstat(CtlS* ctl, int which, u64 n) {
    __hip_atomic_fetch_add(&ctl->st_row[which], n, __ATOMIC_RELAXED, __HIP_MEMORY_SCOPE_WORKGROUP);
}

struct SkView {
    CtlS* ctl; u32* R; u32* U; double* xvals; int* xkeys; u32 MU, MR, CX, shU, shR;
    PushEntry* push2; u32* bt2; int* log_key; unsigned short* log_pu; double* arch;
    u32 lds_u;
    u32* bt_l; u32 bt_l_cap;
};
template <int BLOCK>
__device__ __forceinline__ SkView sk_view(KP p, u32 lds0) {
    SkView w;
    w.MU = 1u << p.sk_lg_mu; w.MR = 1u << p.sk_lg_mr; w.CX = p.sk_cx;
    w.shU = 32u - p.sk_lg_mu; w.shR = 32u - p.sk_lg_mr;
    w.ctl = lds_at<CtlS>(lds0);
    w.R = lds_at<u32>(lds0 + (u32)kCtlBytes);
    w.lds_u = lds0 + (u32)kCtlBytes + 4u * w.MR;
    w.U = lds_at<u32>(w.lds_u);
    w.xvals = lds_at<double>(w.lds_u + 4u * w.MU);
    w.xkeys = lds_at<int>(w.lds_u + 4u * w.MU + 8u * w.CX);
    w.bt_l = lds_at<u32>(lds0 + (u32)kCtlStruct + 64u * kFlatW * (u32)(BLOCK / 64));
    w.bt_l_cap = 16u * kFlatW * (16u - (u32)(BLOCK / 64));
    const u32 wg = blockIdx.x;
    w.push2   = p.push + (u64)(2u * wg) * (u32)p.push_cap;
    w.bt2     = p.bt + (u64)(2u * wg) * (u32)p.bt_cap;
    const u64 log_off = (u64)wg * (u32)p.log_cap;
    w.log_key = p.log_key + log_off;
    w.log_pu  = p.log_pu + log_off;
    w.arch    = p.arch + (u64)wg * (u32)p.arch_cap;
    return w;
}
__device__ __forceinline__ bool sk_res_add_lds(int* keys, double* vals, u32 cap, int k, double v) {
    u32 slot = sk_home((u32)k, cap);
    const int seen = probe_cas_asm(keys, slot, k);
    if (seen != kEmpty && seen != k) return false;
    __hip_atomic_fetch_add(&vals[slot], v, __ATOMIC_RELAXED, __HIP_MEMORY_SCOPE_WORKGROUP);
    return true;
}
__device__ __forceinline__ void sk_insert_window_solo(int* keys, double* vals, u32 cap, u32* flag, int col, double sh, u32& slot, int& seen)
{
    u32 t, h, st; u64 sv, ent;
    slot = 0; seen = 0;
    asm volatile(
        "s_mov_b64 %[sv], exec\n\t"
        "v_cmpx_lt_i32 vcc, -1, %[col]\n\t"
        "s_cbranch_execz 5f\n\t"
        "s_mov_b64 %[ent], exec\n\t"
        "v_mul_u32_u24 %[h], 0x9e3779, %[col]\n\t"
        "v_lshrrev_b32 %[t], 15, %[h]\n\t"
        "v_xor_b32 %[h], %[t], %[h]\n\t"
        "v_mul_u32_u24 %[h], 0x85ebcb, %[h]\n\t"
        "v_lshrrev_b32 %[h], 16, %[h]\n\t"
        "v_mul_u32_u24 %[slot], %[capm], %[h]\n\t"
        "v_lshrrev_b32 %[slot], 16, %[slot]\n\t"
        "s_mov_b32 %[st], 1\n"
        "1:\n\t"
        "v_lshl_add_u32 %[t], %[slot], 2, %[kb]\n\t"
        "ds_cmpst_rtn_b32 %[seen], %[t], %[emp], %[col]\n\t"
        "s_waitcnt lgkmcnt(0)\n\t"
        "v_cmpx_ne_u32 vcc, %[seen], %[col]\n\t"
        "v_cmpx_ne_u32 vcc, -1, %[seen]\n\t"
        "s_cbranch_execz 2f\n\t"
        "v_add_u32 %[slot], %[st], %[slot]\n\t"
        "s_add_u32 %[st], %[st], 1\n\t"
        "s_cmp_le_u32 %[st], %[lim]\n\t"
        "s_cbranch_scc1 1b\n\t"
        "v_mov_b32 %[t], 1\n\t"
        "v_mov_b32 %[h], %[fa]\n\t"
        "ds_write_b32 %[h], %[t]\n"
        "2:\n\t"
        "s_andn2_b64 exec, %[ent], exec\n\t"
        "v_lshl_add_u32 %[t], %[slot], 3, %[vb]\n\t"
        "ds_add_f64 %[t], %[sh]\n"
        "5:\n\t"
        "s_mov_b64 exec, %[sv]"
        : [t] "=&v"(t), [h] "=&v"(h), [slot] "+v"(slot), [seen] "+v"(seen), [sv] "=&s"(sv), [ent] "=&s"(ent), [st] "=&s"(st)
        : [col] "v"(col), [sh] "v"(sh), [emp] "v"(kEmpty),
          [capm] "s"(cap - kProbeSpan), [kb] "s"(lds_addr(keys)), [vb] "s"(lds_addr(vals)), [fa] "s"(lds_addr(flag)), [lim] "n"(kMaxProbe)
        : "vcc", "scc", "memory");
}
__device__ __forceinline__ void lds_add_u32(u32* cell, u32 v) {
    __hip_atomic_fetch_add(cell, v, __ATOMIC_RELAXED, __HIP_MEMORY_SCOPE_WORKGROUP);
}
__device__ __forceinline__ u32 fx_up(double x) { return (u32)__builtin_ceil(x); }

__device__ __forceinline__ u32 sk_degree(KP p, u32 key) {
    const u32 dq = key >> p.deg_shift;
    if (dq != p.deg_sat) return dq;
    const u32 unit = key & p.node_mask;
    if (p.sk_hub_units) return (u32)p.unit_info[unit + 1u];
    const int node = p.unit_info[unit];
    return (u32)(p.indptr[node + 1] - p.indptr[node]);
}

template <bool V> struct SkAllValid { static constexpr bool value = V; };
template <int BLOCK, bool NT = false, class F>
__device__ __forceinline__ void log_groups(const int* lk, const unsigned short* lp, u32 first, u32 end, F f)
{
    typedef int i4 __attribute__((ext_vector_type(4)));
    typedef u32 u2 __attribute__((ext_vector_type(2)));
    constexpr u32 kStride = (BLOCK / 64) * 256u;
    const u32 lane = threadIdx.x & 63u;
    u32 g = (first & ~3u) + wave_id() * 256u;
    if (g >= end) return;
    const u32 last_chunk = (end - 1u) & ~3u;
    i4 kn; u2 pn;
    auto load = [&](u32 g0) {
        const u32 i = min(g0 + 4u * lane, last_chunk);
        if (NT) { kn = __builtin_nontemporal_load((const i4*)&lk[i]); pn = __builtin_nontemporal_load((const u2*)&lp[i]); }
        else    { kn = *(const i4*)&lk[i]; pn = *(const u2*)&lp[i]; }
    };
    load(g);
    for (;;) {
        int k[4]; u32 pu[4];
        const u32 i0 = g + 4u * lane;
        const bool whole = g >= first && g + 256u <= end;
        if (whole) {
#pragma unroll
            for (int q = 0; q < 4; ++q) { k[q] = kn[q]; pu[q] = (pn[q >> 1] >> (16 * (q & 1))) & 0xFFFFu; }
        } else {
#pragma unroll
            for (int q = 0; q < 4; ++q) {
                const bool in = i0 + (u32)q >= first && i0 + (u32)q < end;
                k[q] = in ? kn[q] : -1;
                pu[q] = in ? (pn[q >> 1] >> (16 * (q & 1))) & 0xFFFFu : 0u;
            }
        }
        g += kStride;
        const bool more = g < end;
        if (more) load(g);
// ... 83 lines not shown
        else if (u_next < u_hi) {
            t0n = u_next << kUnitShift; t1n = min(E, min(u_next + 4u, u_hi) << kUnitShift);
            if (!small) {
                const u32 s_no = (u_next - u_lo) >> 2;
                if (s_no - bt_first >= 64u) load_bt(s_no);
                i0n = (u32)__builtin_amdgcn_readlane((int)btv, (int)(s_no - bt_first));
            }
            u_next += 4u;
        } else { have_ent = false; return; }
        if (!small) entn = push[min(i0n + lane, n_ent - 1u)];
    };
    if (small) entn = push[min(lane, n_ent - 1u)];
    fetch_next(0);

    int nc[4] = {-1, -1, -1, -1}; double ns[4] = {0.0, 0.0, 0.0, 0.0}; u32 nu[4] = {0, 0, 0, 0}, nr[4] = {0, 0, 0, 0};
    u32 nt0 = 0;
    bool have_cols = false;
    do {
        u32 idx[4]; double sh[4] = {0.0, 0.0, 0.0, 0.0}; u32 su[4] = {0, 0, 0, 0}, sr[4] = {0, 0, 0, 0}; u32 end = 0;
        if (have_ent) {
            const u32 cnt = min(64u, n_ent - i0n);
            const u32 off = lane < cnt ? entn.off : 0xFFFFFFFFu;
            if (S && lane < cnt) S[i0n + lane] = entn.share;
            end = t1n;
            if (cnt == 64u && i0n + 64u < n_ent) {
                const u32 o63 = (u32)__builtin_amdgcn_readlane((int)off, 63);
                if (o63 < t1n) end = o63;
            }
            *(u32*)(wscr + 4 * lane) = 0u;
            if (off > t0n && off < end) { const u32 pos = off - t0n; wscr[(pos & 63u) * 4u + (pos >> 6)] = 1; }
            asm volatile("" ::: "memory");
            const u32 fl = *(const u32*)(wscr + 4 * lane);
            u32 before = small ? (u32)__popcll(__ballot(off <= t0n)) - 1u : 0u;
            u32 e[4];
#pragma unroll
            for (int w = 0; w < 4; ++w) {
                const bool mine = ((fl >> (8 * w)) & 1u) != 0;
                const u64 M = __ballot(mine);
                e[w] = before + lane_prefix(M) + (mine ? 1u : 0u);
                before += (u32)__popcll(M);
            }
            const u64 sbits = (u64)__double_as_longlong(entn.share);
            u32 eu = 0, er = 0;
            if (FX == 1) eu = fx_up(entn.share * 2147483648.0);
            if (FX != 0) er = fx_up(entn.share * cs);
#pragma unroll
            for (int w = 0; w < 4; ++w) {
                const u32 rel_e = (u32)__builtin_amdgcn_ds_bpermute((int)(e[w] << 2), (int)entn.rel);
                if (FX == 0) {
                    const u32 lo = (u32)__builtin_amdgcn_ds_bpermute((int)(e[w] << 2), (int)(u32)sbits);
                    const u32 hi = (u32)__builtin_amdgcn_ds_bpermute((int)(e[w] << 2), (int)(u32)(sbits >> 32));
                    sh[w] = __longlong_as_double((long long)(((u64)hi << 32) | lo));
                }
                if (FX == 1) su[w] = (u32)__builtin_amdgcn_ds_bpermute((int)(e[w] << 2), (int)eu);
                if (FX != 0) sr[w] = (u32)__builtin_amdgcn_ds_bpermute((int)(e[w] << 2), (int)er);
                const u32 q = t0n + 64u * (u32)w + lane;
                idx[w] = q < end ? rel_e + q : sentinel;
                if (lp && q < end) {
                    const unsigned short pu = (unsigned short)(pu_base + i0n + e[w]);
                    if (NT) __builtin_nontemporal_store(pu, &lp[q]); else lp[q] = pu;
                }
            }
        }
        int cc[4]; double csh[4]; u32 cu[4], cr[4];
#pragma unroll
        for (int w = 0; w < 4; ++w) { cc[w] = nc[w]; csh[w] = ns[w]; cu[w] = nu[w]; cr[w] = nr[w]; }
        const u32 ct0 = nt0;
        const bool had_cols = have_cols;
        have_cols = have_ent;
        if (have_ent) {
#pragma unroll
            for (int w = 0; w < 4; ++w) {
                nc[w] = indices[idx[w]];
                if (FX == 0) ns[w] = sh[w];
                if (FX == 1) nu[w] = su[w];
                if (FX != 0) nr[w] = sr[w];
            }
            nt0 = t0n;
            fetch_next(end);
        }
        if (had_cols) f(cc, csh, cu, cr, ct0);
    } while (have_cols);
}

__device__ __forceinline__ void sk_push_alloc(KP p, CtlS* ctl, LevelCtr* nx, PushEntry* push, u32* bt_g, double* arch, u32 pu_next, double cnext,
                                              u32 len, u32 start, double share, int lane, u32* bt_l, u32 bt_l_cap, u32& n_push, u32& n_edges)
{
    const u64 M = __ballot(len != 0);
    if (M == 0) return;
    const u32 incl = wave_incl_scan_dpp(len);
    const u32 tot = (u32)__builtin_amdgcn_readlane((int)incl, 63);
    n_push += (u32)__popcll(M); n_edges += tot;
    u64 base = 0;
    if (lane == 0)
        base = __hip_atomic_fetch_add(&nx->alloc, ((u64)tot << 32) | (u64)(u32)__popcll(M), __ATOMIC_RELAXED, __HIP_MEMORY_SCOPE_WORKGROUP);
    base = uni(base);
    if (len != 0) {
        const u32 idx = (u32)base + lane_prefix(M), off = (u32)(base >> 32) + (incl - len);
        if ((u64)idx < p.push_cap && (u64)pu_next + idx < p.arch_cap) {
            PushEntry pe; pe.rel = start - off; pe.off = off; pe.share = share; push[idx] = pe;
            arch[pu_next + idx] = cnext * share;
        } else ctl->fail = 1;
        for (u32 m = (off + (1u << kUnitShift) - 1u) >> kUnitShift; ((u64)m << kUnitShift) < (u64)off + len; ++m) {
            if ((u64)m < p.bt_cap) bt_g[m] = idx; else ctl->fail = 1;
            if (m < bt_l_cap) bt_l[m] = idx;
        }
    }
}

template <int BLOCK, int MODE>
__device__ GP_PHASE_NOINLINE void phase_sk_stream(u32 lds0, u32 cur, u32 n_ent, u32 E, u32 seg_base, double cs, u32 capx,
                                                  u32 pu_base, u32 parts, u32 part)
{
    KP p = kparams();
    lds0 = uni(lds0); cur = uni(cur); n_ent = uni(n_ent); E = uni(E); seg_base = uni(seg_base); cs = uni(cs); capx = uni(capx);
    pu_base = uni(pu_base); parts = uni(parts); part = uni(part);
    const SkView w = sk_view<BLOCK>(p, lds0);
    const u32 lane = threadIdx.x & 63u;
    int* lk = w.log_key + seg_base; unsigned short* lp = w.log_pu + seg_base;
    double* S = MODE == 0 ? w.xvals + capx : nullptr;
    const u32* btp = MODE != 3 && ((E + 63u) >> 6) <= w.bt_l_cap ? (const u32*)w.bt_l : (const u32*)(w.bt2 + (u64)cur * (u32)p.bt_cap);
    sk_edge_stream<BLOCK, MODE != 0, MODE == 0 ? 1 : MODE == 2 ? 2 : 0>(p, w.ctl, w.push2 + (u64)cur * (u32)p.push_cap, btp, n_ent, E, S,
                                     MODE != 3 ? lp : nullptr, pu_base, cs,
                                     [&](const int (&v)[4], const double (&sh)[4], const u32 (&su)[4], const u32 (&sr)[4], u32 t0) {
#pragma unroll
        for (int q = 0; q < 4; ++q) {
            if (MODE != 3 && v[q] >= 0) {
                const u32 li = t0 + 64u * (u32)q + lane;
                if (MODE != 0) __builtin_nontemporal_store(v[q], &lk[li]); else lk[li] = v[q];
                const u32 h = sk_cell((u32)v[q]);
                if (cs != 0.0) lds_add_u32(&w.R[h >> w.shR], MODE == 1 ? fx_up(sh[q] * cs) : sr[q]);
                if (MODE == 0) lds_add_u32(&w.U[h >> w.shU], su[q]);
            }
        }
        if (MODE == 1) {
            insert_windows2_asm(w.xkeys, w.xvals, capx, &w.ctl->ovf, v[0], v[1], sh[0], sh[1]);
            insert_windows2_asm(w.xkeys, w.xvals, capx, &w.ctl->ovf, v[2], v[3], sh[2], sh[3]);
        }
        if (MODE == 3) insert_windows4_asm<true>(w.xkeys, w.xvals, capx, &w.ctl->ovf, v, sh, parts, part);
    });
    if (threadIdx.x == 0 && w.ctl->lv_has_dang) {
        const double dang = w.ctl->lv_dang; const int seed_key = w.ctl->seed_key;
        if (MODE != 3) {
            lk[E] = seed_key; lp[E] = (unsigned short)(pu_base + n_ent);
            const u32 h = sk_cell((u32)seed_key);
            if (cs != 0.0) lds_add_u32(&w.R[h >> w.shR], fx_up(dang * cs));
            if (MODE == 0) { lds_add_u32(&w.U[h >> w.shU], fx_up(dang * 2147483648.0)); S[n_ent] = dang; }
        }
        if ((MODE == 1 || (MODE == 3 && (parts == 1u || slot_of(hash_b((u32)seed_key), parts) == part))) &&
            !sk_res_add_lds(w.xkeys, w.xvals, capx, seed_key, dang)) w.ctl->ovf = 1;
    }
}

template <int BLOCK>
__device__ GP_PHASE_NOINLINE void phase_sk_filter(u32 lds0, u32 seg_base, u32 n, u32 capx, u32 pu_base, u32 parts, u32 part)
{
    KP p = kparams();
    lds0 = uni(lds0); seg_base = uni(seg_base); n = uni(n); capx = uni(capx); pu_base = uni(pu_base); parts = uni(parts); part = uni(part);
    const SkView w = sk_view<BLOCK>(p, lds0);
    const float thr = p.sk_thr_f;
    const u32 dshift = (u32)p.deg_shift;
    const double* S = w.xvals + capx;
    u32 n_cand = 0;
    SKT2(w.ctl, 0);
    log_groups<BLOCK>(w.log_key, w.log_pu, seg_base, seg_base + n, [&](const int (&k)[4], const u32 (&pu)[4], auto all_valid) {
        constexpr bool kAll = decltype(all_valid)::value;
        u32 cell[4]; double s[4];
#pragma unroll
        for (int q = 0; q < 4; ++q) {
            cell[q] = w.U[sk_cell(kAll ? (u32)k[q] : (u32)max(k[q], 0)) >> w.shU];
            s[q] = S[kAll || k[q] >= 0 ? pu[q] - pu_base : 0u];
        }
        int kc[4];
#pragma unroll
        for (int q = 0; q < 4; ++q) {
            const u32 dq = (u32)k[q] >> dshift;
            const bool cand = (kAll || k[q] >= 0) && (float)cell[q] >= (float)dq * thr;
            n_cand += (u32)__popcll(__ballot(cand));
            kc[q] = cand ? k[q] : -1;
        }
        insert_windows4_asm<true>(w.xkeys, w.xvals, capx, &w.ctl->ovf, kc, s, parts, part);
    });
    if ((threadIdx.x & 63u) == 0 && n_cand && part == 0u) zstat(w.ctl, zCand, n_cand);
    SKT2(w.ctl, 1);
}

template <int BLOCK>
__device__ GP_PHASE_NOINLINE void phase_sk_scan(u32 lds0, u32 cap, u32 nx_sel, u32 nxt_sel, u32 clear_n, u32 pu_next, double cnext)
{
    typedef int    i4 __attribute__((ext_vector_type(4)));
    typedef double d2 __attribute__((ext_vector_type(2)));
    typedef u32    u4 __attribute__((ext_vector_type(4)));
    KP p = kparams();
    lds0 = uni(lds0); cap = uni(cap); nx_sel = uni(nx_sel); nxt_sel = uni(nxt_sel); clear_n = uni(clear_n); pu_next = uni(pu_next); cnext = uni(cnext);
    const SkView w = sk_view<BLOCK>(p, lds0);
    CtlS* ctl = w.ctl;
    int* lkeys = w.xkeys; double* lvals = w.xvals;
    const u32 C = w.CX;
    LevelCtr* nx = &ctl->lc[nx_sel];
    PushEntry* push = w.push2 + (u64)nxt_sel * (u32)p.push_cap;
    u32* bt_g = w.bt2 + (u64)nxt_sel * (u32)p.bt_cap;
    const int tid = threadIdx.x, lane = tid & 63;
    SKT2(ctl, 4);
    if (clear_n) {
        const u4 z = {0u, 0u, 0u, 0u};
        for (u32 i = 4u * (u32)tid; i < w.MU; i += 4u * BLOCK) *(u4*)&w.U[i] = z;
        for (u32 i = (u32)tid; i < clear_n; i += BLOCK) lvals[cap + i] = 0.0;
    }
    constexpr u32 kWaves = BLOCK / 64;
    const u32 range = ((cap + kWaves * 256u - 1u) / (kWaves * 256u)) * 256u;
    const u32 wb = wave_id() * range;
    u32 tot = 0, ncand = 0;
    const double rmax_ = p.rmax; const u32 dsh = (u32)p.deg_shift;
    for (u32 sub = wb; sub < wb + range && sub < cap; sub += 256u) {
        const u32 s0 = sub + 4u * (u32)lane;
        i4 kk = {kEmpty, kEmpty, kEmpty, kEmpty};
        if (s0 < cap) kk = *(const i4*)&lkeys[s0];
        const bool o0 = kk.x != kEmpty, o1 = kk.y != kEmpty, o2 = kk.z != kEmpty, o3 = kk.w != kEmpty;
        const u32 n_occ = (u32)__popcll(__ballot(o0)) + (u32)__popcll(__ballot(o1)) + (u32)__popcll(__ballot(o2)) + (u32)__popcll(__ballot(o3));
        if (n_occ == 0) continue;
        tot += n_occ;
        d2 ra = {0.0, 0.0}, rb = {0.0, 0.0};
        if (o0 | o1 | o2 | o3) {
            ra = *(const d2*)&lvals[s0]; rb = *(const d2*)&lvals[s0 + 2];
            const i4 ke = {kEmpty, kEmpty, kEmpty, kEmpty};
            const d2 z = {0.0, 0.0};
            *(i4*)&lkeys[s0] = ke; *(d2*)&lvals[s0] = z; *(d2*)&lvals[s0 + 2] = z;
        }
        __atomic_signal_fence(__ATOMIC_SEQ_CST);
        const u32 d0 = (u32)kk.x >> dsh, d1 = (u32)kk.y >> dsh, d2_ = (u32)kk.z >> dsh, d3 = (u32)kk.w >> dsh;
        const bool c0b = o0 && (d0 == 0u || ra.x >= rmax_ * (double)d0), c1b = o1 && (d1 == 0u || ra.y >= rmax_ * (double)d1),
                   c2b = o2 && (d2_ == 0u || rb.x >= rmax_ * (double)d2_), c3b = o3 && (d3 == 0u || rb.y >= rmax_ * (double)d3);
        const u64 m0 = __ballot(c0b), m1 = __ballot(c1b), m2 = __ballot(c2b), m3 = __ballot(c3b);
        const u32 c0 = (u32)__popcll(m0), c1 = (u32)__popcll(m1), c2 = (u32)__popcll(m2), c3 = (u32)__popcll(m3);
        const u32 q0 = wb + ncand;
        if (c0b) { const u32 q = q0 + lane_prefix(m0);                lkeys[q] = kk.x; lvals[q] = ra.x; }
        if (c1b) { const u32 q = q0 + c0 + lane_prefix(m1);           lkeys[q] = kk.y; lvals[q] = ra.y; }
        if (c2b) { const u32 q = q0 + c0 + c1 + lane_prefix(m2);      lkeys[q] = kk.z; lvals[q] = rb.x; }
        if (c3b) { const u32 q = q0 + c0 + c1 + c2 + lane_prefix(m3); lkeys[q] = kk.w; lvals[q] = rb.y; }
        __atomic_signal_fence(__ATOMIC_SEQ_CST);
        ncand += c0 + c1 + c2 + c3;
    }
    (void)C;
    u32 st_push = 0, st_edges = 0, st_deg = 0;
    SKT2(ctl, 5);
    if (tot != 0) {
        SKT2(ctl, 6);
        for (u32 j = 0; j < ncand; j += 64u) {
            const u32 idx = j + (u32)lane;
            const bool want = idx < ncand;
            int k = kEmpty; double r = 0.0; u32 deg = 0;
            if (want) {
                k = lkeys[wb + idx]; r = lvals[wb + idx];
                lkeys[wb + idx] = kEmpty; lvals[wb + idx] = 0.0;
                deg = (u32)k >> p.deg_shift;
                if (deg == p.deg_sat) deg = sk_degree(p, (u32)k);
            }
            double share = 0.0; u32 len = 0;
            if (want) {
                if (deg == 0) {
                    __hip_atomic_fetch_add(&nx->dangling, r, __ATOMIC_RELAXED, __HIP_MEMORY_SCOPE_WORKGROUP);
                    __hip_atomic_fetch_add(&nx->n_dangling, 1u, __ATOMIC_RELAXED, __HIP_MEMORY_SCOPE_WORKGROUP);
                } else if (r >= p.rmax * (double)deg) {
                    const double sh = r / (double)deg;
                    if (sh != 0.0) { share = sh; len = deg; }
                }
            }
            st_deg += (u32)__popcll(__ballot(want && ((u32)k >> p.deg_shift) == p.deg_sat));
            sk_push_alloc(p, ctl, nx, push, bt_g, w.arch, pu_next, cnext, len, ((u32)k & p.node_mask) << kSkUnitShift, share, lane, w.bt_l, w.bt_l_cap, st_push, st_edges);
        }
        SKT2(ctl, 7);
        if (lane == 0) {
            __hip_atomic_fetch_add(&nx->n_rec, tot, __ATOMIC_RELAXED, __HIP_MEMORY_SCOPE_WORKGROUP);
            if (st_deg) zstat(ctl, zDeg, st_deg);
            if (st_push) { zstat(ctl, zPush, st_push); zstat(ctl, zEdges, st_edges); }
        }
    }
    SKT2(ctl, 8);
}

constexpr u32 kSkSoloEdges = 256;
template <int BLOCK, bool SEED = false>
__device__ GP_PHASE_NOINLINE void phase_sk_solo(u32 lds0, u32 cur, u32 n_ent, u32 E, u32 seg_base, double cs,
                                                u32 has_dang, double dang, int seed_key, u32 nx_sel, u32 pu_base, u32 pu_next, double cnext,
                                                u32 seed_rel = 0, double seed_share = 0.0)
{
    KP p = kparams();
    lds0 = uni(lds0); cur = uni(cur); n_ent = uni(n_ent); E = uni(E); seg_base = uni(seg_base); cs = uni(cs);
    has_dang = uni(has_dang); dang = uni(dang); seed_key = uni(seed_key); nx_sel = uni(nx_sel);
    pu_base = uni(pu_base); pu_next = uni(pu_next); cnext = uni(cnext);
    const SkView w = sk_view<BLOCK>(p, lds0);
    CtlS* ctl = w.ctl; int* lkeys = w.xkeys; double* lvals = w.xvals;
    const u32 lane = threadIdx.x & 63u;
    const u32 cap = kMinCap;
    const SerialSection ahead;
    unsigned char* wscr = (unsigned char*)ctl + kCtlStruct;
    u32* list = (u32*)((unsigned char*)ctl + kCtlStruct + 64 * kFlatW);
    static_assert((BLOCK / 64 - 1) * 64 * kFlatW >= 4 * (kSkSoloEdges + 1), "the claimed-slot list lives in the parked waves' flag bytes");
    LevelCtr* nx = &ctl->lc[nx_sel];
    const PushEntry* push_cur = w.push2 + (u64)cur * (u32)p.push_cap;
    PushEntry* push_nxt = w.push2 + (u64)(cur ^ 1u) * (u32)p.push_cap;
    u32* bt_nxt = w.bt2 + (u64)(cur ^ 1u) * (u32)p.bt_cap;
    int* lk = w.log_key + seg_base; unsigned short* lp = w.log_pu + seg_base;
    PushEntry ent;
    if (SEED) { ent.rel = uni(seed_rel); ent.off = 0u; ent.share = uni(seed_share); }
    else ent = push_cur[min(lane, n_ent - 1u)];
    const u32 off = lane < n_ent ? ent.off : 0xFFFFFFFFu;
    *(u32*)(wscr + 4 * lane) = 0u;
    if (off > 0u && off < E) wscr[(off & 63u) * 4u + (off >> 6)] = 1;
    asm volatile("" ::: "memory");
    const u32 fl = *(const u32*)(wscr + 4 * lane);
    u32 before = (u32)__popcll(__ballot(off == 0u)) - 1u;
    int col[4]; double sh[4]; u32 own[4];
    {
        const u64 sbits = (u64)__double_as_longlong(ent.share);
#pragma unroll
        for (int q = 0; q < 4; ++q) {
            const bool mine = ((fl >> (8 * q)) & 1u) != 0;
            const u64 M = __ballot(mine);
            own[q] = before + lane_prefix(M) + (mine ? 1u : 0u);
            before += (u32)__popcll(M);
        }
#pragma unroll
        for (int q = 0; q < 4; ++q) {
            const u32 rel_e = (u32)__builtin_amdgcn_ds_bpermute((int)(own[q] << 2), (int)ent.rel);
            const u32 lo = (u32)__builtin_amdgcn_ds_bpermute((int)(own[q] << 2), (int)(u32)sbits);
            const u32 hi = (u32)__builtin_amdgcn_ds_bpermute((int)(own[q] << 2), (int)(u32)(sbits >> 32));
            const u32 eq = 64u * (u32)q + lane;
            col[q] = p.indices[eq < E ? rel_e + eq : (u32)p.nnz];
            sh[q] = __longlong_as_double((long long)(((u64)hi << 32) | lo));
        }
    }
    u32 n_list = 0;
#pragma unroll
    for (int q = 0; q < 5; ++q) {
        if (q == 4 && !has_dang) break;
        const int kq = q < 4 ? col[q] : (lane == 0 ? seed_key : -1);
        const double vq = q < 4 ? sh[q] : dang;
        if (kq >= 0) {
            const u32 li = q < 4 ? 64u * (u32)q + lane : E;
            __builtin_nontemporal_store(kq, &lk[li]);
            __builtin_nontemporal_store((unsigned short)(pu_base + (q < 4 ? own[q < 4 ? q : 0] : n_ent)), &lp[li]);
            if (cs != 0.0) lds_add_u32(&w.R[sk_cell((u32)kq) >> w.shR], fx_up(vq * cs));
        }
        u32 slot; int seen;
        sk_insert_window_solo(lkeys, lvals, cap, &ctl->ovf, kq, vq, slot, seen);
        const bool fresh = kq >= 0 && seen == kEmpty;
        const u64 M = __ballot(fresh);
        if (fresh) list[n_list + lane_prefix(M)] = slot;
        n_list += (u32)__popcll(M);
    }
    asm volatile("" ::: "memory");
    if (uni(ctl->ovf)) {
        for (u32 j = lane; j < n_list; j += 64u) { const u32 sl = list[j]; lkeys[sl] = kEmpty; lvals[sl] = 0.0; }
        if (lane == 0) GP_OVF_COUNT(p, kOvfSolo);
        return;
    }
    u32 st_push = 0, st_edges = 0, st_deg = 0;
    for (u32 j = 0; j < n_list; j += 64u) {
        const bool valid = j + lane < n_list;
        int k = kEmpty; double r = 0.0;
// ... 41 lines not shown
    t.CA = sk_top_slots(region_bytes, n_pu, (u32)p.K);
    t.T = lds_at<double>(w.lds_u);
    const u32 a0 = w.lds_u + 8u * ((n_pu + 1u) & ~1u);
    t.avals = lds_at<double>(a0);
    t.akeys = lds_at<int>(a0 + 8u * t.CA);
    t.tie = lds_at<Cand>(a0 + 12u * t.CA);
    t.sel = t.tie + kSkTie;
    t.fine = (u32*)((unsigned char*)w.ctl + kCtlStruct);
    return t;
}

template <int BLOCK>
__device__ __forceinline__ void sk_rank_selected(KP p, CtlS* ctl, const SkTop& t, u32 need, bool take_all, u32& my_rank)
{
    const int tid = threadIdx.x;
    if (!take_all) {
        const u32 nt = uni(ctl->n_tie), n0 = uni(ctl->n_sel), want = need - n0;
        for (u32 i = tid; i < nt; i += BLOCK) {
            Cand mine = t.tie[i];
            const int mk = (int)((u32)mine.key & p.node_mask);
            u32 rank = 0;
            for (u32 j = 0; j < nt; ++j) {
                const Cand o = t.tie[j];
                const int ok = (int)((u32)o.key & p.node_mask);
                rank += (o.bits > mine.bits || (o.bits == mine.bits && ok < mk)) ? 1u : 0u;
            }
            if (rank < want) t.sel[n0 + rank] = mine;
        }
        GP_SYNC();
    }
    if ((u32)tid < need) {
        const Cand cd = t.sel[tid];
        const int ck = (int)((u32)cd.key & p.node_mask);
        u32 rank = 0;
        for (u32 j = 0; j < need; ++j) {
            const Cand o = t.sel[j];
            const int ok = (int)((u32)o.key & p.node_mask);
            rank += (o.bits > cd.bits || (o.bits == cd.bits && ok < ck)) ? 1u : 0u;
        }
        my_rank = rank;
        if (rank + 1u == need) ctl->kth_bits = cd.bits;
    }
    GP_SYNC();
}

constexpr u32 kSkNarrow = 16;
template <class F>
__device__ __forceinline__ void sk_table_walk(const SkTop& t, int block, F f)
{
    typedef int    i4 __attribute__((ext_vector_type(4)));
    typedef double d2 __attribute__((ext_vector_type(2)));
    for (u32 s0 = 4u * threadIdx.x; s0 < t.CA; s0 += 4u * (u32)block) {
        const i4 kk = *(const i4*)&t.akeys[s0];
        if (kk.x == kEmpty && kk.y == kEmpty && kk.z == kEmpty && kk.w == kEmpty) continue;
        const d2 va = *(const d2*)&t.avals[s0], vb = *(const d2*)&t.avals[s0 + 2];
        if (kk.x != kEmpty && va.x > 0.0) f(kk.x, (u64)__double_as_longlong(va.x));
        if (kk.y != kEmpty && va.y > 0.0) f(kk.y, (u64)__double_as_longlong(va.y));
        if (kk.z != kEmpty && vb.x > 0.0) f(kk.z, (u64)__double_as_longlong(vb.x));
        if (kk.w != kEmpty && vb.y > 0.0) f(kk.w, (u64)__double_as_longlong(vb.y));
    }
}
template <int BLOCK>
__device__ __forceinline__ u32 sk_select(KP p, CtlS* ctl, const SkTop& t, u32& my_rank)
{
    const int tid = threadIdx.x, lane = tid & 63;
    const u32 K = (u32)p.K;
    sk_table_walk(t, BLOCK, [&](int, u64 bits) {
        const int e = 1023 - (int)(bits >> 52);
        if ((u32)e < 64u) lds_add_u32(&ctl->bcnt[e], 1u); else ctl->tk_wide = 1u;
    });
    GP_SYNC();
    if (uni(ctl->tk_wide)) return 0xFFFFFFFFu;
    u32 above, cnt_b, b_sel, need;
    {
        const u32 cn = ctl->bcnt[lane];
        const u32 incl = wave_incl_scan_dpp(cn);
        const u32 total = (u32)__builtin_amdgcn_readlane((int)incl, 63);
        need = min(K, total);
        if (need == 0) return 0;
        const u64 mk = __ballot(incl >= need);
        b_sel = (u32)(__ffsll((long long)mk) - 1);
        above = (u32)__builtin_amdgcn_readlane((int)(incl - cn), (int)b_sel);
        cnt_b = (u32)__builtin_amdgcn_readlane((int)cn, (int)b_sel);
    }
    u32 vshift = 52; u64 vpre = (u64)(1023u - b_sel);
    u32 ishift = 8u * (u32)(((int)p.deg_shift + 7) / 8), ipre = 0, buf = 0;
    while (above + cnt_b > need && cnt_b > kSkNarrow && (vshift > 0u || ishift > 0u)) {
        const bool by_value = vshift > 0u;
        const u32 ds = by_value ? min(8u, vshift) : 8u;
        const u32 vs_hi = vshift, is_hi = ishift;
        if (by_value) vshift -= ds; else ishift -= ds;
        u32* fine = t.fine + 256u * buf; buf ^= 1u;
        for (u32 i = tid; i < 256u; i += BLOCK) fine[i] = 0;
        GP_SYNC();
        sk_table_walk(t, BLOCK, [&](int key, u64 bits) {
            const u32 id = (u32)key & p.node_mask;
            if ((bits >> vs_hi) == vpre && (by_value || is_hi >= 32u || (id >> is_hi) == ipre)) {
                const u32 dg = by_value ? (u32)(bits >> vshift) & ((1u << ds) - 1u) : (id >> ishift) & 255u;
                lds_add_u32(&fine[by_value ? 255u - dg : dg], 1u);
            }
        });
        GP_SYNC();
        {
            u32 c4[4], sum = 0;
#pragma unroll
            for (int j = 0; j < 4; ++j) { c4[j] = fine[4 * lane + j]; sum += c4[j]; }
            const u32 incl = wave_incl_scan_dpp(sum) + above;
            const u64 m = __ballot(incl >= need);
            const int cl = m ? __ffsll((long long)m) - 1 : 63;
            u32 acc = incl - sum, cj = c4[3]; int js = 3;
#pragma unroll
            for (int j = 0; j < 4; ++j) { if (acc + c4[j] >= need) { js = j; cj = c4[j]; break; } acc += c4[j]; }
            const u32 bin = 4u * (u32)cl + (u32)__builtin_amdgcn_readlane(js, cl);
            above = (u32)__builtin_amdgcn_readlane((int)acc, cl);
            cnt_b = (u32)__builtin_amdgcn_readlane((int)cj, cl);
            if (by_value) vpre = (vpre << ds) | (u64)(255u - bin); else ipre = (ipre << 8) | bin;
        }
    }
    if (above + cnt_b > need && cnt_b > kSkTie) return 0xFFFFFFFFu;
    const bool take_all = above + cnt_b <= need;
    {
        typedef int    i4 __attribute__((ext_vector_type(4)));
        typedef double d2 __attribute__((ext_vector_type(2)));
        for (u32 base = 0; base < t.CA; base += 4u * BLOCK) {
            const u32 s0 = base + 4u * (u32)tid;
            i4 kk = {kEmpty, kEmpty, kEmpty, kEmpty}; d2 va = {0.0, 0.0}, vb = {0.0, 0.0};
            if (s0 < t.CA) { kk = *(const i4*)&t.akeys[s0]; va = *(const d2*)&t.avals[s0]; vb = *(const d2*)&t.avals[s0 + 2]; }
            const double v[4] = {va.x, va.y, vb.x, vb.y};
#pragma unroll
            for (int j = 0; j < 4; ++j) {
                if (__ballot(kk[j] != kEmpty && v[j] > 0.0) == 0) continue;
                bool is_sel = false, is_t = false;
                Cand cd; cd.bits = (u64)__double_as_longlong(v[j]); cd.key = kk[j]; cd.pad = 0;
                if (kk[j] != kEmpty && v[j] > 0.0) {
                    const u32 id = (u32)cd.key & p.node_mask;
                    const u64 vbits = cd.bits >> vshift;
                    const bool v_eq = vbits == vpre;
                    const bool in_bin = v_eq && (ishift >= 32u || (id >> ishift) == ipre);
                    const bool over = vbits > vpre || (v_eq && ishift < 32u && (id >> ishift) < ipre);
                    is_sel = over || (in_bin && take_all); is_t = in_bin && !take_all;
                }
                const u32 si = wave_alloc1(&ctl->n_sel, is_sel, lane);
                if (is_sel) t.sel[si] = cd;
                const u32 ti = wave_alloc1(&ctl->n_tie, is_t, lane);
                if (is_t) t.tie[ti] = cd;
            }
        }
    }
    GP_SYNC();
    sk_rank_selected<BLOCK>(p, ctl, t, need, take_all, my_rank);
    return need;
}

template <int BLOCK, bool TG>
__device__ GP_PHASE_NOINLINE void phase_sk_topk(u32 lds0, u32 row_lo, u32 row_hi, int seed, u32 n_pu, u32 n_log)
{
    KP p = kparams();
    lds0 = uni(lds0); row_lo = uni(row_lo); row_hi = uni(row_hi); seed = uni(seed); n_pu = uni(n_pu); n_log = uni(n_log);
    const SkView w = sk_view<BLOCK>(p, lds0);
    CtlS* ctl = w.ctl;
    const SkTop t = sk_top(p, w, TG ? 0u : n_pu);
    const long long row = (long long)(((u64)row_hi << 32) | row_lo);
    const int tid = threadIdx.x, lane = tid & 63;
    const u32 wave = wave_id();
    const u32 K = (u32)p.K;

    if (!TG) for (u32 i = tid; i < n_pu; i += BLOCK) t.T[i] = w.arch[i];
    for (u32 i = tid; i < 512u; i += BLOCK) t.fine[i] = 0;
    for (u32 i = tid; i < t.CA; i += BLOCK) { t.akeys[i] = kEmpty; t.avals[i] = 0.0; }
    if (tid < 64) ctl->bcnt[tid] = 0;
    if (tid == 0) { ctl->ovf = 0; ctl->tk_t = 1u; ctl->n_sel = 0; ctl->n_tie = 0; ctl->tk_wide = 0; ctl->kth_bits = ~0ull; }
    bool table_ready = true;
    GP_SYNC();
    for (u32 i = tid; i < t.MR; i += BLOCK) {
        const u32 cv = t.R[i];
        if (cv) {
            const u32 fb = __float_as_uint((float)cv);
            lds_add_u32(&t.fine[min(511u, (fb >> 19) - (127u << 4))], 1u);
        }
    }
    GP_SYNC();
    u32 t_c;
    {
        u32 cnt8[8], sum = 0;
#pragma unroll
        for (int j = 0; j < 8; ++j) { cnt8[j] = t.fine[8 * lane + j]; sum += cnt8[j]; }
        const u32 suf = wave_suffix_scan(sum, lane);
        const u64 m = __ballot(suf >= p.sk_target);
        u32 edge = 1u;
        if (m != 0) {
            const int cl = 63 - __builtin_clzll(m);
            u32 acc = suf - sum; int js = 0;
#pragma unroll
            for (int j = 7; j >= 0; --j) { acc += cnt8[j]; if (acc >= p.sk_target) { js = j; break; } }
            const u32 bin = 8u * (u32)cl + (u32)__builtin_amdgcn_readlane(js, cl), e = bin >> 4, mt = 16u + (bin & 15u);
            edge = max(e >= 4u ? mt << (e - 4u) : mt >> (4u - e), 1u);
        }
        t_c = edge;
    }
    SKT(ctl, 7);
    u32 need = 0, my_rank = 0;
    bool last = false;
    for (int round = 0; ; ++round) {
        u32 P = 1;
        for (;;) {
            bool ovf = false;
            for (u32 part = 0; part < P; ++part) {
                const u32 n_run = part == 0 ? 0u : need;
                Cand mine; mine.bits = 0; mine.key = kEmpty; mine.pad = 0;
                if ((u32)tid < n_run) mine = t.sel[tid];
                if (!table_ready) {
                    GP_SYNC();
                    for (u32 i = tid; i < t.CA; i += BLOCK) { t.akeys[i] = kEmpty; t.avals[i] = 0.0; }
                    if (tid < 64) ctl->bcnt[tid] = 0;
                    if (tid == 0) { ctl->n_sel = 0; ctl->n_tie = 0; ctl->tk_wide = 0; ctl->kth_bits = ~0ull; }
                    GP_SYNC();
                }
                table_ready = false;
                if (n_run != 0u) {
                    if (mine.key != kEmpty) { t.akeys[t.CA - 1u - (u32)tid] = mine.key; t.avals[t.CA - 1u - (u32)tid] = __longlong_as_double((long long)mine.bits); }
                    GP_SYNC();
                }
                auto tabled = [&](const int (&k)[4], const u32 (&pu)[4], auto all_valid) {
                    constexpr bool kAll = decltype(all_valid)::value;
                    u32 cell[4]; double cv[4];
#pragma unroll
                    for (int q = 0; q < 4; ++q) {
                        cell[q] = t.R[sk_cell(kAll ? (u32)k[q] : (u32)max(k[q], 0)) >> t.shR];
                        cv[q] = TG ? w.arch[pu[q]] : t.T[pu[q]];
                    }
                    int kh[4];
#pragma unroll
                    for (int q = 0; q < 4; ++q) kh[q] = (kAll || k[q] >= 0) && cv[q] != 0.0 && cell[q] >= t_c ? k[q] : -1;
                    insert_windows4_asm<true>(t.akeys, t.avals, t.CA, &ctl->ovf, kh, cv, P, part);
                };
#if GP_SK_SWEEP_DEPTH == 2
                log_groups2_nt<BLOCK>(w.log_key, w.log_pu, n_log, tabled);
#else
                log_groups<BLOCK, true>(w.log_key, w.log_pu, 0u, n_log, tabled);
#endif
                GP_SYNC();
                SKT(ctl, 8);
                if (uni(ctl->ovf)) { ovf = true; break; }
                need = sk_select<BLOCK>(p, ctl, t, my_rank);
                SKT(ctl, 9);
                if (need == 0xFFFFFFFFu) { if (tid == 0) ctl->fail = 3; GP_SYNC(); return; }
            }
            if (!ovf) break;
            GP_SYNC();
            if (tid == 0) { ctl->ovf = 0; GP_OVF_COUNT(p, kOvfTopk); }
            P *= 2; need = 0;
            if (P > 64u) { if (tid == 0) ctl->fail = 4; GP_SYNC(); return; }
            GP_SYNC();
        }
        if (t_c <= 1u || last) break;
        if (need == K) {
            const double tau_fx = __builtin_floor(__longlong_as_double((long long)uni(ctl->kth_bits)) * p.sk_rscale * (1.0 - 1.0 / 1048576.0));
            if (tau_fx >= (double)t_c) break;
            t_c = tau_fx >= 1.0 ? (u32)tau_fx : 1u;
            last = true;
        } else {
            t_c = round >= 2 ? 1u : max(1u, t_c >> 4);
        }
        if (tid == 0) zstat(ctl, zSweep2, 1);
    }
    const long long out0 = row * (long long)p.K;
    if ((u32)tid < need) {
        const Cand cd = t.sel[tid];
        const int node = p.unit_info[(u32)cd.key & p.node_mask];
        __builtin_nontemporal_store(seed, &p.out_row[out0 + my_rank]);
        __builtin_nontemporal_store(node, &p.out_col[out0 + my_rank]);
        __builtin_nontemporal_store(__longlong_as_double((long long)cd.bits), &p.out_val[out0 + my_rank]);
    }
    publish_filled(p, row, need);
    if (tid == 0) zstat(ctl, zFilled, need);
}

template <int BLOCK>
__device__ GP_PHASE_NOINLINE void phase_sk_wipe(u32 lds0, u32 what, u32 n, u32 at)
{
    typedef u32 u4 __attribute__((ext_vector_type(4)));
    KP p = kparams();
    lds0 = uni(lds0); what = uni(what); n = uni(n); at = uni(at);
    const SkView w = sk_view<BLOCK>(p, lds0);
    const u4 z = {0u, 0u, 0u, 0u};
    if (what == 1u) {
        for (u32 i = 4u * threadIdx.x; i < w.MR + w.MU; i += 4u * BLOCK) *(u4*)&w.R[i] = z;
        n = w.CX;
    }
    if (what == 3u) {
        for (u32 i = 4u * threadIdx.x; i < w.MU; i += 4u * BLOCK) *(u4*)&w.U[i] = z;
        for (u32 i = threadIdx.x; i < n; i += BLOCK) w.xvals[at + i] = 0.0;
        return;
    }
    for (u32 i = threadIdx.x; i < n; i += BLOCK) { w.xkeys[i] = kEmpty; w.xvals[i] = 0.0; }
}

__device__ __forceinline__ u64 sk_io_pack(u32 pu_next, u32 log_next) { return ((u64)log_next << 32) | pu_next; }

template <int BLOCK>
__device__ GP_PHASE_NOINLINE u32 phase_sk_seed(u32 lds0, int seed)
{
    KP p = kparams();
    lds0 = uni(lds0); seed = uni(seed);
    const SkView w = sk_view<BLOCK>(p, lds0);
    CtlS* ctl = w.ctl;
    const int tid = threadIdx.x;
    const u32 L = (u32)p.n_coef - 1u;
    const u32 seed_unit = uni(p.node_pos[seed]);
    const u32 seed_deg = uni((u32)p.indptr[seed + 1]) - uni((u32)p.indptr[seed]);
    const u32 s_start = seed_unit << kSkUnitShift;
    const int seed_key = (int)(seed_unit | (min(seed_deg, p.deg_sat) << p.deg_shift));
    const u32 pu_cap = (u32)min((u64)kSkMaxPushers, p.arch_cap);
    PushEntry* push1 = w.push2 + (u64)(u32)p.push_cap;
    u32* bt1 = w.bt2 + (u64)(u32)p.bt_cap;
    const bool room = p.log_cap > 0 && pu_cap >= 2u && p.push_cap > 0;
    bool pushes = false; double share = 0.0;
    if (L > 0 && seed_deg != 0 && 1.0 >= p.rmax * (double)seed_deg) {
        share = 1.0 / (double)seed_deg;
        pushes = share != 0.0;
        if (tid == 0) { zstat(ctl, zPush, 1); zstat(ctl, zEdges, seed_deg); }
    }
    const u32 units = (seed_deg + (1u << kUnitShift) - 1u) >> kUnitShift;
    const u32 k_lc = uni(ctl->k_log_cap), k_so = uni(ctl->k_solo_ok), k_dm = uni(ctl->k_direct_max);
    const bool merged = (p.solo & 2u) != 0u && k_so != 0u && pushes && room && L >= 2u && seed_deg <= kSkSoloEdges && seed_deg <= k_dm &&
                        (u64)units <= p.bt_cap && (u64)1u + seed_deg <= (u64)k_lc && (u64)2u + kSkSoloEdges + 4u <= (u64)pu_cap;
    if (merged && wave_id() != 0u) return 1u;
    if (tid == 0) {
        ctl->seed_key = seed_key; ctl->tot_pu = 1; ctl->tot_log = 1;
        if (room) { w.log_key[0] = seed_key; w.log_pu[0] = 0; w.arch[0] = ctl->coef[0]; }
        if (!room || (pushes && (u64)units > p.bt_cap)) ctl->fail = 1;
        lds_add_u32(&w.R[sk_cell((u32)seed_key) >> w.shR], fx_up(ctl->coef[0] * p.sk_rscale));
        zstat(ctl, zLevels, 1);
        LevelCtr* l0 = &ctl->lc[0];
        l0->dangling = L > 0 && seed_deg == 0 ? 1.0 : 0.0; l0->n_dangling = L > 0 && seed_deg == 0 ? 1u : 0u;
        l0->n_rec = 0; l0->alloc = pushes ? ((u64)seed_deg << 32) | 1ull : 0ull; l0->pad1 = sk_io_pack(1u, 1u);
        if (pushes && room) {
            PushEntry pe; pe.rel = s_start; pe.off = 0; pe.share = share; push1[0] = pe;
            w.arch[1] = ctl->coef[1] * share;
        }
    }
    if (pushes && (u64)units <= p.bt_cap)
        for (u32 m = (u32)tid; m < units; m += BLOCK) { bt1[m] = 0u; if (m < w.bt_l_cap) w.bt_l[m] = 0u; }
    if (!merged) return 0u;
    if (tid == 0) {
        LevelCtr* nx = &ctl->lc[1];
        nx->dangling = 0.0; nx->n_dangling = 0; nx->n_rec = 0; nx->alloc = 0ull; nx->pad1 = sk_io_pack(2u, 1u + seed_deg);
        ctl->tot_pu = 2u; ctl->tot_log = 1u + seed_deg; ctl->max_e = max(ctl->max_e, seed_deg);
        ctl->lv_has_dang = 0u; ctl->lv_dang = 0.0;
        zstat(ctl, zLevels, 1);
    }
    __atomic_signal_fence(__ATOMIC_SEQ_CST);
    phase_sk_solo<BLOCK, true>(lds0, 1u, 1u, seed_deg, 1u, ctl->coef[1] * ctl->k_rscale, 0u, 0.0, seed_key, 1u, 1u, 2u, ctl->coef[2], s_start, share);
    return 1u;
}

template <int BLOCK, bool REDO = false>
__device__ __forceinline__ u32 phase_sk_level(u32 lds0, u32 lvl, u32 L)
{
    KP p = kparams();
    lds0 = uni(lds0); lvl = uni(lvl); L = uni(L);
    const SkView w = sk_view<BLOCK>(p, lds0);
    CtlS* ctl = w.ctl;
    const int tid = threadIdx.x;
    const LevelCtr* in = &ctl->lc[(lvl & 1u) ^ 1u];
    LevelCtr* nx = &ctl->lc[lvl & 1u];
    const u64 al_ = in->alloc, io_ = in->pad1; const u32 nd_ = in->n_dangling, fail_ = ctl->fail, q_ = ctl->cand_q[lvl]; const int sk_ = ctl->seed_key;
    const double dg_ = in->dangling, c_ = ctl->coef[lvl], c1_ = ctl->coef[lvl + 1u], krs_ = ctl->k_rscale;
    const u32 klc_ = ctl->k_log_cap, kpc_ = ctl->k_pu_cap, kdm_ = ctl->k_direct_max, kso_ = ctl->k_solo_ok, kcx_ = ctl->k_cx;
    const u32 CX = uni(kcx_);
    const u64 al = uni(al_), io = uni(io_);
    const u32 n_ent_cur = (u32)al, e_cur = (u32)(al >> 32), pu_cur = (u32)io, log_pos = (u32)(io >> 32);
    const bool has_dang_cur = uni(nd_) != 0u;
    const double dang_cur = has_dang_cur ? uni(dg_) : 0.0;
    const int seed_key = uni(sk_);
    const u32 n_rec = e_cur + (has_dang_cur ? 1u : 0u);
    if (n_rec == 0 || uni(fail_)) return 0u;
    const bool last = lvl == L;
    const u32 pu_cap = uni(kpc_);
    if ((u64)log_pos + n_rec > (u64)uni(klc_) || (u64)pu_cur + n_ent_cur + 1u > pu_cap) { if (tid == 0) ctl->fail = 1; return 0u; }
    const u32 seg_base = log_pos;
    const u32 pu_next = pu_cur + n_ent_cur + (has_dang_cur ? 1u : 0u);
    const u32 cur = lvl & 1u;
    if (tid == 0) {
        nx->dangling = 0.0; nx->n_dangling = 0; nx->n_rec = 0; nx->alloc = 0ull; nx->pad1 = sk_io_pack(pu_next, log_pos + n_rec);
        ctl->tot_pu = pu_next; ctl->tot_log = log_pos + n_rec; ctl->max_e = max(ctl->max_e, e_cur);
        ctl->lv_has_dang = has_dang_cur ? 1u : 0u; ctl->lv_dang = dang_cur;
        if (has_dang_cur) w.arch[pu_cur + n_ent_cur] = uni(c_) * dang_cur;
        if (!REDO) zstat(ctl, zLevels, 1);
    }
    const double cs = uni(c_) * uni(krs_);
    const double cnext = last ? 0.0 : uni(c1_);
    SKT(ctl, 6);
    if (last) {
        phase_sk_stream<BLOCK, 2>(lds0, cur, n_ent_cur, e_cur, seg_base, cs, 0u, pu_cur, 1u, 0u);
        SKT(ctl, 3);
        return 0u;
    }
    const u32 direct_max = uni(kdm_);
    const u32 s_n = n_ent_cur + 1u;
    const bool direct = n_rec <= direct_max || s_n + kMinCap > CX;
    u32 capx = direct ? min(CX, max(kMinCap, (4u * n_rec + 3u) & ~3u)) : (CX - s_n) & ~3u;
    const u32 cap0 = capx;
    u32 P0 = 1;
    {
        const u32 q = uni(q_);
        const u32 est = direct ? (n_rec > direct_max ? 2u * n_rec : 0u) : (u32)(((u64)n_rec * q) >> 10);
        while (P0 < 64u && est > P0 * capx) ++P0;
    }
    const bool solo = !REDO && uni(kso_) && direct && e_cur <= kSkSoloEdges && n_ent_cur >= 1u && n_ent_cur <= 64u &&
                      (u64)pu_next + kSkSoloEdges + 4u <= pu_cap;
    if (REDO) {
    } else if (solo) {
        if (wave_id() == 0)
            phase_sk_solo<BLOCK>(lds0, cur, n_ent_cur, e_cur, seg_base, cs, has_dang_cur ? 1u : 0u, dang_cur, seed_key, lvl & 1u, pu_cur, pu_next, cnext);
        GP_SYNC();
        SKT(ctl, 1); SKT_COUNT(ctl, 13, 1);
    } else {
        SKT2_BEGIN(ctl);
        if (direct && P0 == 1u) phase_sk_stream<BLOCK, 1>(lds0, cur, n_ent_cur, e_cur, seg_base, cs, capx, pu_cur, 1u, 0u);
        else if (direct)        phase_sk_stream<BLOCK, 2>(lds0, cur, n_ent_cur, e_cur, seg_base, cs, capx, pu_cur, 1u, 0u);
        else                    phase_sk_stream<BLOCK, 0>(lds0, cur, n_ent_cur, e_cur, seg_base, cs, capx, pu_cur, 1u, 0u);
        SKT2(ctl, 11);
        GP_SYNC();
        SKT2(ctl, 12);
        SKT(ctl, direct ? 1 : 2); SKT_COUNT(ctl, direct ? 13 : 14, 1);
    }
    const bool by_log = !direct;
    bool u_dirty = !direct, first = true;
    u32 part = 0, np = P0;
    bool level_done = false;
    if (solo) {
        if (!uni(ctl->ovf)) level_done = true;
        else { capx = CX; }
    }
    if (REDO) capx = CX;
    if (!level_done)
    for (;;) {
        if (!(first && direct && P0 == 1u)) {
            SKT2_BEGIN(ctl);
            if (by_log) phase_sk_filter<BLOCK>(lds0, seg_base, n_rec, capx, pu_cur, np, part);
            else        phase_sk_stream<BLOCK, 3>(lds0, cur, n_ent_cur, e_cur, seg_base, cs, capx, pu_cur, np, part);
            SKT2(ctl, 2);
            GP_SYNC();
            SKT2(ctl, 3);
            SKT(ctl, 4); SKT_COUNT(ctl, 11, 1);
        }
        first = false;
        if (uni(ctl->ovf)) {
            phase_sk_wipe<BLOCK>(lds0, 2u, by_log ? cap0 : CX, 0u);
            GP_SYNC();
            if (tid == 0) { ctl->ovf = 0; GP_OVF_COUNT(p, kOvfLevel); }
            if (!by_log) capx = CX;
            if (np < 0x10000u) { part *= 2; np *= 2; GP_SYNC(); continue; }
            if (tid == 0) ctl->fail = 5;
            GP_SYNC();
            break;
        }
        const bool final_part = np == P0 && part + 1u == P0;
        SKT2_BEGIN(ctl);
        phase_sk_scan<BLOCK>(lds0, capx, lvl & 1u, cur ^ 1u, final_part && u_dirty ? s_n : 0u, pu_next, cnext);
        if (final_part) u_dirty = false;
        SKT2(ctl, 9);
        GP_SYNC();
        SKT2(ctl, 10);
        SKT(ctl, 5); SKT_COUNT(ctl, 12, 1);
        if (uni(ctl->fail)) break;
        while (np > P0 && (part & 1u)) { part >>= 1; np >>= 1; }
        ++part;
        if (np == P0 && part == P0) break;
    }
    if (u_dirty) {
        phase_sk_wipe<BLOCK>(lds0, 3u, s_n, cap0);
        GP_SYNC();
    }
    if (uni(ctl->fail)) return 0u;
    if (tid == 0 && !direct) {
        const u32 obs = min(2048u, (u32)(1280.0f * (float)nx->n_rec * __frcp_rn((float)n_rec)) + 8u);
        const u32 old_q = ctl->cand_q[lvl];
        ctl->cand_q[lvl] = max(obs, old_q - (old_q >> 3));
    }
    return 1u;
}

template <int BLOCK>
__device__ GP_PHASE_NOINLINE u32 phase_sk_level1_redo(u32 lds0, u32 L) { return phase_sk_level<BLOCK, true>(lds0, 1u, L); }

template <int BLOCK>
__device__ __forceinline__ void gfpush_sk_rows()
{
    extern __shared__ __attribute__((aligned(16))) unsigned char smem[];
    KP p = kparams();
    const u32 lds0 = uni(lds_addr(smem));
    const SkView w = sk_view<BLOCK>(p, lds0);
    CtlS* ctl = w.ctl;
    const int tid = threadIdx.x;
    phase_sk_wipe<BLOCK>(lds0, 1u, 0u, 0u);
    if (tid < 8) { ctl->st[tid] = 0; ctl->st_row[tid] = 0; }
#ifdef GP_SK_TIMING
    if (tid < 16) ctl->tacc[tid] = 0;
    if (tid < 14) ctl->tacc2[tid] = 0;
    if (tid < 32) ctl->row_hist[tid] = 0;
    if (tid == 0) { ctl->t_enter = wall_clock64(); ctl->row_sum = 0; ctl->row_max = 0; }
#endif
    if (tid < kSkMaxCoef) { ctl->cand_q[tid] = 0; if (tid < p.n_coef) ctl->coef[tid] = p.coef[tid]; }
    if (tid == 0) {
        ctl->max_e = 0; ctl->max_log = 0;
        ctl->k_log_cap = (u32)min(p.log_cap, (u64)0xFFFFFFFFu); ctl->k_pu_cap = (u32)min((u64)kSkMaxPushers, p.arch_cap);
        ctl->k_direct_max = min(p.sk_direct_max, 3u * (w.CX / 4u)); ctl->k_cx = w.CX; ctl->k_rscale = p.sk_rscale;
        ctl->k_solo_ok = (p.solo & 1u) && p.push_cap >= (u64)kSkSoloEdges + 4u &&
                         (double)p.bt_cap >= (p.rmax > 0.0 ? fmin((double)p.nnz, 1.001 / p.rmax + 16.0) : (double)p.nnz) / (double)(1u << kUnitShift) + 4.0 ? 1u : 0u;
    }
    const long long n_rows = p.n_seeds;
    const u32 L = (u32)p.n_coef - 1u;

    for (;;) {
        GP_SYNC();
        SKT_BEGIN(ctl);
        if (tid == 0) {
            long long q = (long long)__hip_atomic_fetch_add(&p.counters[p.queue_counter], 1ull, __ATOMIC_RELAXED, __HIP_MEMORY_SCOPE_AGENT);
            if (p.row_map && q < n_rows) q = (long long)p.row_map[q];
            ctl->row = q;
            ctl->fail = 0; ctl->ovf = 0;
#ifdef GP_SK_TIMING
            ctl->t_row = ctl->tlast;
#endif
        }
        GP_SYNC();
        const long long row = uni(ctl->row);
        if (row >= n_rows) break;
        const int seed = uni(p.seeds[row]);
        if (seed < 0 || seed >= p.n_nodes) {
            if (tid == 0) { __hip_atomic_fetch_add(&ctl->st[zFailed], 1ull, __ATOMIC_RELAXED, __HIP_MEMORY_SCOPE_WORKGROUP); if (p.out_filled) p.out_filled[row] = 0; }
            continue;
        }
        u32 lvl = 1u + uni(phase_sk_seed<BLOCK>(lds0, seed));
        GP_SYNC();
        SKT(ctl, 0); SKT_COUNT(ctl, 15, 1);
        if (lvl == 2u) {
            SKT_COUNT(ctl, 13, 1);
            if (uni(ctl->ovf)) lvl = uni(phase_sk_level1_redo<BLOCK>(lds0, L)) ? 2u : L + 1u;
        }
        for (; lvl <= L; ++lvl)
            if (!uni(phase_sk_level<BLOCK>(lds0, lvl, L))) break;
        GP_SYNC();
        SKT(ctl, 6);
        if (!uni(ctl->fail)) {
            const u32 n_pu = uni(ctl->tot_pu), n_log = uni(ctl->tot_log);
            if (tid == 0) ctl->max_log = max(ctl->max_log, n_log);
            const u32 top_region = 4u * w.MU + 12u * w.CX;
            if (2u * sk_top_slots(top_region, n_pu, (u32)p.K) >= sk_top_slots(top_region, 0u, (u32)p.K))
                 phase_sk_topk<BLOCK, false>(lds0, (u32)(u64)row, (u32)((u64)row >> 32), seed, n_pu, n_log);
            else phase_sk_topk<BLOCK, true>(lds0, (u32)(u64)row, (u32)((u64)row >> 32), seed, n_pu, n_log);
        }
        GP_SYNC();
        if (uni(ctl->fail)) {
            if (tid == 0) {
                const u64 i = __hip_atomic_fetch_add(&p.counters[p.retry_counter], 1ull, __ATOMIC_RELAXED, __HIP_MEMORY_SCOPE_AGENT);
                p.retry_list[i] = (u32)row;
                if (ctl->fail == 1) __hip_atomic_fetch_add(&p.counters[kSkSlabFails], 1ull, __ATOMIC_RELAXED, __HIP_MEMORY_SCOPE_AGENT);
#ifndef GP_SK_TIMING
                __hip_atomic_fetch_add(&p.counters[kDiag0 + min(ctl->fail, 7u)], 1ull, __ATOMIC_RELAXED, __HIP_MEMORY_SCOPE_AGENT);
#endif
            }
            if (tid < 8) ctl->st_row[tid] = 0;
        } else if (tid < 8) { ctl->st[tid] += ctl->st_row[tid]; ctl->st_row[tid] = 0; }
        GP_SYNC();
        phase_sk_wipe<BLOCK>(lds0, 1u, 0u, 0u);
        SKT(ctl, 10);
#ifdef GP_SK_TIMING
        if (tid == 0) {
            const u64 dt = ctl->tlast - ctl->t_row;
            ctl->row_sum += dt; ctl->row_max = max(ctl->row_max, dt); ++ctl->row_hist[min(31u, 63u - (u32)__builtin_clzll(dt | 1ull))];
        }
#endif
    }
#ifdef GP_SK_TIMING
    if (tid == 0 && p.wg_log) { p.wg_log[2u * blockIdx.x] = ctl->t_enter; p.wg_log[2u * blockIdx.x + 1u] = wall_clock64(); }
#endif
    GP_SYNC();
    if (tid == 0) {
        const Counter dst[zNumStats] = { kPushes, kEdges, kDegLookups, kFilled, kLdsLevels, kFailedRows, kSkCandEdges, kSkSweep2 };
#pragma unroll
        for (int i = 0; i < zNumStats; ++i)
            if (ctl->st[i]) __hip_atomic_fetch_add(&p.counters[dst[i]], ctl->st[i], __ATOMIC_RELAXED, __HIP_MEMORY_SCOPE_AGENT);
        if (ctl->max_e) __hip_atomic_fetch_max(&p.counters[kMaxLevelEdges], (u64)ctl->max_e, __ATOMIC_RELAXED, __HIP_MEMORY_SCOPE_AGENT);
        if (ctl->max_log) __hip_atomic_fetch_max(&p.counters[kMaxLogRecords], (u64)ctl->max_log, __ATOMIC_RELAXED, __HIP_MEMORY_SCOPE_AGENT);
#ifdef GP_SK_TIMING
        for (int i = 0; i < 16; ++i) __hip_atomic_fetch_add(&p.counters[kDiag0 + i], ctl->tacc[i], __ATOMIC_RELAXED, __HIP_MEMORY_SCOPE_AGENT);
        for (int i = 0; i < 14; ++i) __hip_atomic_fetch_add(&p.counters[kDiagX0 + i], ctl->tacc2[i], __ATOMIC_RELAXED, __HIP_MEMORY_SCOPE_AGENT);
        __hip_atomic_fetch_add(&p.counters[kDiagX0 + 16], ctl->row_sum, __ATOMIC_RELAXED, __HIP_MEMORY_SCOPE_AGENT);
        __hip_atomic_fetch_max(&p.counters[kDiagX0 + 17], ctl->row_max, __ATOMIC_RELAXED, __HIP_MEMORY_SCOPE_AGENT);
        for (int i = 0; i < 32; ++i)
            if (ctl->row_hist[i]) __hip_atomic_fetch_add(&p.counters[kDiagX0 + 32 + i], ctl->row_hist[i], __ATOMIC_RELAXED, __HIP_MEMORY_SCOPE_AGENT);
#endif
    }
}

template <int BLOCK>
__global__ void __launch_bounds__(BLOCK, BLOCK == 1024 ? 4 : 6) gfpush_sk_kernel(const KParams)
{
    gfpush_sk_rows<BLOCK>();
}

}

#endif
```

Before: 3.595 million.

## Add compacted candidate list for multi-part sketch filter and top-k passes

Adds an opt-in sk_cand_list option. When a sketch level or top-k pass overflows and must be split into hash partitions, the first partitioned pass writes the keys that belong to other partitions into a compact list, and later partitions walk only that list instead of the whole log. It also moves the overflow and partition retry paths into separate noinline redo functions (level redo, topk_parts) so the common single-part path stays lean, and separates clearing of U from clearing of S. The list path is off by default. The split hot path and redo restructuring run by default and trade some code size and extra atomics for less re-scanning in overflow cases.

Result: no change. 3.577 million (-0.5%).

```diff
diff --git a/grand_plus_amd/csrc/gfpush.hip b/grand_plus_amd/csrc/gfpush.hip
--- a/grand_plus_amd/csrc/gfpush.hip
+++ b/grand_plus_amd/csrc/gfpush.hip
@@ -557,7 +557,8 @@
     kp.prune = prune_allowed(g->opt, a.coef, a.n_coef) ? 1 : 0;
     kp.diag_flags = g->opt.diag_flags;
     kp.rows_distinct = g->rows_distinct && g->opt.seedrow ? 1u : 0u;
-    kp.solo = (g->opt.solo_levels ? 1u : 0u) | (g->opt.sk_seed_merge ? 2u : 0u);
+    kp.solo = (g->opt.solo_levels ? 1u : 0u) | (g->opt.sk_seed_merge ? 2u : 0u) |
+              (g->opt.sk_cand_list ? 4u : 0u);
     kp.direct = direct_tables(g->opt, g->n_nodes, gk) ? 1 : 0;
     return kp;
 }
@@ -1053,6 +1054,8 @@
         g->opt.sk_direct_max = (int)value;
     } else if (k == "sk_seed_merge") {
         g->opt.sk_seed_merge = value ? 1 : 0;
+    } else if (k == "sk_cand_list") {
+        g->opt.sk_cand_list = value ? 1 : 0;
     } else if (k == "row_order") {
         g->opt.row_order = value ? 1 : 0;
     } else if (k == "gk_acsr") {
@@ -1329,7 +1332,7 @@
     q->opt.block_threads = src->opt.block_threads; q->opt.lds_bytes = src->opt.lds_bytes; q->opt.max_workgroups = src->opt.max_workgroups;
     q->opt.workspace_mb = src->opt.workspace_mb; q->opt.force_global = src->opt.force_global; q->opt.exact_stats = src->opt.exact_stats;
     q->opt.direct_tables = src->opt.direct_tables; q->opt.est_level_edges = src->opt.est_level_edges; q->opt.seedrow = src->opt.seedrow; q->opt.solo_levels = src->opt.solo_levels;
-    q->opt.kernel = src->opt.kernel; q->opt.row_order = src->opt.row_order; q->opt.gk_acsr = src->opt.gk_acsr; q->opt.sk_seed_merge = src->opt.sk_seed_merge; q->opt.sk_block = src->opt.sk_block; q->opt.sk_lg_mu = src->opt.sk_lg_mu; q->opt.sk_lg_mr = src->opt.sk_lg_mr; q->opt.sk_target = src->opt.sk_target; q->opt.lds_pad = src->opt.lds_pad; q->opt.sk_direct_max = src->opt.sk_direct_max;
+    q->opt.kernel = src->opt.kernel; q->opt.row_order = src->opt.row_order; q->opt.gk_acsr = src->opt.gk_acsr; q->opt.sk_seed_merge = src->opt.sk_seed_merge; q->opt.sk_cand_list = src->opt.sk_cand_list; q->opt.sk_block = src->opt.sk_block; q->opt.sk_lg_mu = src->opt.sk_lg_mu; q->opt.sk_lg_mr = src->opt.sk_lg_mr; q->opt.sk_target = src->opt.sk_target; q->opt.lds_pad = src->opt.lds_pad; q->opt.sk_direct_max = src->opt.sk_direct_max;
     const size_t b_ptr = sizeof(int) * (size_t)(q->n_nodes + 1), b_idx = sizeof(int) * (size_t)(q->nnz + 1);
     HIP_TRY(hipMalloc(&q->d_indptr, b_ptr));
     HIP_TRY(hipMalloc(&q->d_indices, b_idx));
diff --git a/grand_plus_amd/csrc/gfpush_kernels.hpp b/grand_plus_amd/csrc/gfpush_kernels.hpp
--- a/grand_plus_amd/csrc/gfpush_kernels.hpp
+++ b/grand_plus_amd/csrc/gfpush_kernels.hpp
@@ -156,12 +156,15 @@
 
 enum OvfCount { kOvfLevel = 8,
                 kOvfSolo = 9,
-                kOvfTopk = 10 };
+                kOvfTopk = 10,
+                kSkListed = 11,
+                kSkListWalks = 12 };
 #if !defined(GP_DIAG) && !defined(GP_SK_TIMING)
-#define GP_OVF_COUNT(p, which) __hip_atomic_fetch_add(&(p).counters[kDiag0 + (which)], 1ull, __ATOMIC_RELAXED, __HIP_MEMORY_SCOPE_AGENT)
+#define GP_OVF_ADD(p, which, n) __hip_atomic_fetch_add(&(p).counters[kDiag0 + (which)], (u64)(n), __ATOMIC_RELAXED, __HIP_MEMORY_SCOPE_AGENT)
 #else
-#define GP_OVF_COUNT(p, which) do { } while (0)
-#endif
+#define GP_OVF_ADD(p, which, n) do { } while (0)
+#endif
+#define GP_OVF_COUNT(p, which) GP_OVF_ADD(p, which, 1u)
 
 #ifdef GP_DIAG_HEAVY
 constexpr int kSyncBase = __COUNTER__;
diff --git a/grand_plus_amd/csrc/gfpush_plan.hpp b/grand_plus_amd/csrc/gfpush_plan.hpp
--- a/grand_plus_amd/csrc/gfpush_plan.hpp
+++ b/grand_plus_amd/csrc/gfpush_plan.hpp
@@ -30,6 +30,7 @@
     int sk_block = 0, sk_lg_mu = 0, sk_lg_mr = 0, sk_target = 0, sk_direct_max = 0;
     int row_order = 1;
     int sk_seed_merge = 1; int gk_acsr = 1;
+    int sk_cand_list = 0;
     int64_t est_level_edges = 0;
     int measure_choice = 1;
     int max_degree_bits = 31;
diff --git a/grand_plus_amd/csrc/gfpush_sketch.hpp b/grand_plus_amd/csrc/gfpush_sketch.hpp
--- a/grand_plus_amd/csrc/gfpush_sketch.hpp
+++ b/grand_plus_amd/csrc/gfpush_sketch.hpp
@@ -28,7 +28,7 @@
     int seed_key; u32 tot_pu, tot_log;
     double lv_dang; u32 lv_has_dang;
     u32 max_e, max_log;
-    u32 k_log_cap, k_pu_cap, k_direct_max, k_solo_ok, k_cx, k_pad; double k_rscale;
+    u32 k_log_cap, k_pu_cap, k_direct_max, k_solo_ok, k_cx, n_list; double k_rscale;
 #ifdef GP_SK_TIMING
     u64 tacc[16]; u64 tlast;
     u64 tacc2[14]; u64 tlast2;
@@ -418,11 +418,12 @@
     }
 }
 
-template <int BLOCK>
-__device__ GP_PHASE_NOINLINE void phase_sk_filter(u32 lds0, u32 seg_base, u32 n, u32 capx, u32 pu_base, u32 parts, u32 part)
+template <int BLOCK, int LIST>
+__device__ GP_PHASE_NOINLINE void phase_sk_filter(u32 lds0, u32 seg_base, u32 n, u32 capx, u32 pu_base, u32 parts, u32 part, u32 list_base)
 {
     KP p = kparams();
     lds0 = uni(lds0); seg_base = uni(seg_base); n = uni(n); capx = uni(capx); pu_base = uni(pu_base); parts = uni(parts); part = uni(part);
+    list_base = uni(list_base);
     const SkView w = sk_view<BLOCK>(p, lds0);
     const float thr = p.sk_thr_f;
     const u32 dshift = (u32)p.deg_shift;
@@ -434,31 +435,54 @@
         u32 cell[4]; double s[4];
 #pragma unroll
         for (int q = 0; q < 4; ++q) {
-            cell[q] = w.U[sk_cell(kAll ? (u32)k[q] : (u32)max(k[q], 0)) >> w.shU];
+            if (LIST != 2) cell[q] = w.U[sk_cell(kAll ? (u32)k[q] : (u32)max(k[q], 0)) >> w.shU];
             s[q] = S[kAll || k[q] >= 0 ? pu[q] - pu_base : 0u];
         }
         int kc[4];
-#pragma unroll
-        for (int q = 0; q < 4; ++q) {
-            const u32 dq = (u32)k[q] >> dshift;
-            const bool cand = (kAll || k[q] >= 0) && (float)cell[q] >= (float)dq * thr;
-            n_cand += (u32)__popcll(__ballot(cand));
-            kc[q] = cand ? k[q] : -1;
+        if (LIST == 2) {
+#pragma unroll
+            for (int q = 0; q < 4; ++q) kc[q] = k[q];
+        } else {
+            u64 ml[4]; u32 n_l = 0;
+#pragma unroll
+            for (int q = 0; q < 4; ++q) {
+                const u32 dq = (u32)k[q] >> dshift;
+                const bool cand = (kAll || k[q] >= 0) && (float)cell[q] >= (float)dq * thr;
+                n_cand += (u32)__popcll(__ballot(cand));
+                kc[q] = cand ? k[q] : -1;
+                if (LIST == 1) {
+                    ml[q] = __ballot(cand && slot_of(hash_b((u32)k[q]), parts) != part);
+                    n_l += (u32)__popcll(ml[q]);
+                }
+            }
+            if (LIST == 1 && n_l != 0u) {
+                u32 at = 0;
+                if ((threadIdx.x & 63u) == 0u) at = __hip_atomic_fetch_add(&w.ctl->n_list, n_l, __ATOMIC_RELAXED, __HIP_MEMORY_SCOPE_WORKGROUP);
+                at = list_base + uni(at);
+#pragma unroll
+                for (int q = 0; q < 4; ++q) {
+                    if ((ml[q] >> (threadIdx.x & 63u)) & 1ull) {
+                        const u32 i = at + lane_prefix(ml[q]);
+                        w.log_key[i] = k[q]; w.log_pu[i] = (unsigned short)pu[q];
+                    }
+                    at += (u32)__popcll(ml[q]);
+                }
+            }
         }
         insert_windows4_asm<true>(w.xkeys, w.xvals, capx, &w.ctl->ovf, kc, s, parts, part);
     });
-    if ((threadIdx.x & 63u) == 0 && n_cand && part == 0u) zstat(w.ctl, zCand, n_cand);
+    if (LIST != 2 && (threadIdx.x & 63u) == 0 && n_cand && part == 0u) zstat(w.ctl, zCand, n_cand);
     SKT2(w.ctl, 1);
 }
 
 template <int BLOCK>
-__device__ GP_PHASE_NOINLINE void phase_sk_scan(u32 lds0, u32 cap, u32 nx_sel, u32 nxt_sel, u32 clear_n, u32 pu_next, double cnext)
+__device__ GP_PHASE_NOINLINE void phase_sk_scan(u32 lds0, u32 cap, u32 nx_sel, u32 nxt_sel, u32 clear_u, u32 clear_n, u32 pu_next, double cnext)
 {
     typedef int    i4 __attribute__((ext_vector_type(4)));
     typedef double d2 __attribute__((ext_vector_type(2)));
     typedef u32    u4 __attribute__((ext_vector_type(4)));
     KP p = kparams();
-    lds0 = uni(lds0); cap = uni(cap); nx_sel = uni(nx_sel); nxt_sel = uni(nxt_sel); clear_n = uni(clear_n); pu_next = uni(pu_next); cnext = uni(cnext);
+    lds0 = uni(lds0); cap = uni(cap); nx_sel = uni(nx_sel); nxt_sel = uni(nxt_sel); clear_u = uni(clear_u); clear_n = uni(clear_n); pu_next = uni(pu_next); cnext = uni(cnext);
     const SkView w = sk_view<BLOCK>(p, lds0);
     CtlS* ctl = w.ctl;
     int* lkeys = w.xkeys; double* lvals = w.xvals;
@@ -468,11 +492,11 @@
     u32* bt_g = w.bt2 + (u64)nxt_sel * (u32)p.bt_cap;
     const int tid = threadIdx.x, lane = tid & 63;
     SKT2(ctl, 4);
-    if (clear_n) {
+    if (clear_u) {
         const u4 z = {0u, 0u, 0u, 0u};
         for (u32 i = 4u * (u32)tid; i < w.MU; i += 4u * BLOCK) *(u4*)&w.U[i] = z;
-        for (u32 i = (u32)tid; i < clear_n; i += BLOCK) lvals[cap + i] = 0.0;
-    }
+    }
+    for (u32 i = (u32)tid; i < clear_n; i += BLOCK) lvals[cap + i] = 0.0;
     constexpr u32 kWaves = BLOCK / 64;
     const u32 range = ((cap + kWaves * 256u - 1u) / (kWaves * 256u)) * 256u;
     const u32 wb = wave_id() * range;
@@ -820,8 +844,75 @@
     return need;
 }
 
+template <int BLOCK, bool TG, int LIST>
+__device__ GP_PHASE_NOINLINE void phase_sk_topk_part(u32 lds0, u32 n_pu, u32 first, u32 end, u32 t_c, u32 P, u32 part, u32 list_base)
+{
+    KP p = kparams();
+    lds0 = uni(lds0); n_pu = uni(n_pu); first = uni(first); end = uni(end); t_c = uni(t_c); P = uni(P); part = uni(part); list_base = uni(list_base);
+    const SkView w = sk_view<BLOCK>(p, lds0);
+    CtlS* ctl = w.ctl;
+    const SkTop t = sk_top(p, w, TG ? 0u : n_pu);
+    const u32 lane = threadIdx.x & 63u;
+    auto tabled = [&](const int (&k)[4], const u32 (&pu)[4], auto all_valid) {
+        constexpr bool kAll = decltype(all_valid)::value;
+        u32 cell[4]; double cv[4];
+#pragma unroll
+        for (int q = 0; q < 4; ++q) {
+            cell[q] = t.R[sk_cell(kAll ? (u32)k[q] : (u32)max(k[q], 0)) >> t.shR];
+            cv[q] = TG ? w.arch[kAll || k[q] >= 0 ? pu[q] : 0u] : t.T[kAll || k[q] >= 0 ? pu[q] : 0u];
+        }
+        int kh[4]; u64 ml[4]; u32 n_l = 0;
+#pragma unroll
+        for (int q = 0; q < 4; ++q) {
+            kh[q] = (kAll || k[q] >= 0) && cv[q] != 0.0 && cell[q] >= t_c ? k[q] : -1;
+            if (LIST == 1) {
+                ml[q] = __ballot(kh[q] >= 0 && slot_of(hash_b((u32)kh[q]), P) != part);
+                n_l += (u32)__popcll(ml[q]);
+            }
+        }
+        if (LIST == 1 && n_l != 0u) {
+            u32 at = 0;
+            if (lane == 0u) at = __hip_atomic_fetch_add(&ctl->n_list, n_l, __ATOMIC_RELAXED, __HIP_MEMORY_SCOPE_WORKGROUP);
+            at = list_base + uni(at);
+#pragma unroll
+            for (int q = 0; q < 4; ++q) {
+                if ((ml[q] >> lane) & 1ull) {
+                    const u32 i = at + lane_prefix(ml[q]);
+                    w.log_key[i] = k[q]; w.log_pu[i] = (unsigned short)pu[q];
+                }
+                at += (u32)__popcll(ml[q]);
+            }
+        }
+        insert_windows4_asm<true>(t.akeys, t.avals, t.CA, &ctl->ovf, kh, cv, P, part);
+    };
+    if (LIST == 2) log_groups<BLOCK>(w.log_key, w.log_pu, first, end, tabled);
+#if GP_SK_SWEEP_DEPTH == 2
+    else log_groups2_nt<BLOCK>(w.log_key, w.log_pu, end, tabled);
+#else
+    else log_groups<BLOCK, true>(w.log_key, w.log_pu, first, end, tabled);
+#endif
+}
+
+__device__ __forceinline__ void sk_write_row(KP p, CtlS* ctl, const SkTop& t, long long row, int seed, u32 need, u32 my_rank)
+{
+    const int tid = threadIdx.x;
+    const long long out0 = row * (long long)p.K;
+    if ((u32)tid < need) {
+        const Cand cd = t.sel[tid];
+        const int node = p.unit_info[(u32)cd.key & p.node_mask];
+        __builtin_nontemporal_store(seed, &p.out_row[out0 + my_rank]);
+        __builtin_nontemporal_store(node, &p.out_col[out0 + my_rank]);
+        __builtin_nontemporal_store(__longlong_as_double((long long)cd.bits), &p.out_val[out0 + my_rank]);
+    }
+    publish_filled(p, row, need);
+    if (tid == 0) zstat(ctl, zFilled, need);
+}
+
 template <int BLOCK, bool TG>
-__device__ GP_PHASE_NOINLINE void phase_sk_topk(u32 lds0, u32 row_lo, u32 row_hi, int seed, u32 n_pu, u32 n_log)
+__device__ GP_PHASE_NOINLINE u32 phase_sk_topk_parts(u32 lds0, u32 row_lo, u32 row_hi, int seed, u32 n_pu, u32 n_log);
+
+template <int BLOCK, bool TG>
+__device__ GP_PHASE_NOINLINE u32 phase_sk_topk(u32 lds0, u32 row_lo, u32 row_hi, int seed, u32 n_pu, u32 n_log)
 {
     KP p = kparams();
     lds0 = uni(lds0); row_lo = uni(row_lo); row_hi = uni(row_hi); seed = uni(seed); n_pu = uni(n_pu); n_log = uni(n_log);
@@ -870,57 +961,43 @@
     u32 need = 0, my_rank = 0;
     bool last = false;
     for (int round = 0; ; ++round) {
-        u32 P = 1;
-        for (;;) {
-            bool ovf = false;
-            for (u32 part = 0; part < P; ++part) {
-                const u32 n_run = part == 0 ? 0u : need;
-                Cand mine; mine.bits = 0; mine.key = kEmpty; mine.pad = 0;
-                if ((u32)tid < n_run) mine = t.sel[tid];
-                if (!table_ready) {
-                    GP_SYNC();
-                    for (u32 i = tid; i < t.CA; i += BLOCK) { t.akeys[i] = kEmpty; t.avals[i] = 0.0; }
-                    if (tid < 64) ctl->bcnt[tid] = 0;
-                    if (tid == 0) { ctl->n_sel = 0; ctl->n_tie = 0; ctl->tk_wide = 0; ctl->kth_bits = ~0ull; }
-                    GP_SYNC();
-                }
-                table_ready = false;
-                if (n_run != 0u) {
-                    if (mine.key != kEmpty) { t.akeys[t.CA - 1u - (u32)tid] = mine.key; t.avals[t.CA - 1u - (u32)tid] = __longlong_as_double((long long)mine.bits); }
-                    GP_SYNC();
-                }
-                auto tabled = [&](const int (&k)[4], const u32 (&pu)[4], auto all_valid) {
-                    constexpr bool kAll = decltype(all_valid)::value;
-                    u32 cell[4]; double cv[4];
-#pragma unroll
-                    for (int q = 0; q < 4; ++q) {
-                        cell[q] = t.R[sk_cell(kAll ? (u32)k[q] : (u32)max(k[q], 0)) >> t.shR];
-                        cv[q] = TG ? w.arch[pu[q]] : t.T[pu[q]];
-                    }
-                    int kh[4];
-#pragma unroll
-                    for (int q = 0; q < 4; ++q) kh[q] = (kAll || k[q] >= 0) && cv[q] != 0.0 && cell[q] >= t_c ? k[q] : -1;
-                    insert_windows4_asm<true>(t.akeys, t.avals, t.CA, &ctl->ovf, kh, cv, P, part);
-                };
+        if (!table_ready) {
+            GP_SYNC();
+            for (u32 i = tid; i < t.CA; i += BLOCK) { t.akeys[i] = kEmpty; t.avals[i] = 0.0; }
+            if (tid < 64) ctl->bcnt[tid] = 0;
+            if (tid == 0) { ctl->n_sel = 0; ctl->n_tie = 0; ctl->tk_wide = 0; ctl->kth_bits = ~0ull; }
+            GP_SYNC();
+        }
+        table_ready = false;
+        auto tabled = [&](const int (&k)[4], const u32 (&pu)[4], auto all_valid) {
+            constexpr bool kAll = decltype(all_valid)::value;
+            u32 cell[4]; double cv[4];
+#pragma unroll
+            for (int q = 0; q < 4; ++q) {
+                cell[q] = t.R[sk_cell(kAll ? (u32)k[q] : (u32)max(k[q], 0)) >> t.shR];
+                cv[q] = TG ? w.arch[pu[q]] : t.T[pu[q]];
+            }
+            int kh[4];
+#pragma unroll
+            for (int q = 0; q < 4; ++q) kh[q] = (kAll || k[q] >= 0) && cv[q] != 0.0 && cell[q] >= t_c ? k[q] : -1;
+            insert_windows4_asm<true>(t.akeys, t.avals, t.CA, &ctl->ovf, kh, cv, 1u, 0u);
+        };
 #if GP_SK_SWEEP_DEPTH == 2
-                log_groups2_nt<BLOCK>(w.log_key, w.log_pu, n_log, tabled);
+        log_groups2_nt<BLOCK>(w.log_key, w.log_pu, n_log, tabled);
 #else
-                log_groups<BLOCK, true>(w.log_key, w.log_pu, 0u, n_log, tabled);
+        log_groups<BLOCK, true>(w.log_key, w.log_pu, 0u, n_log, tabled);
 #endif
-                GP_SYNC();
-                SKT(ctl, 8);
-                if (uni(ctl->ovf)) { ovf = true; break; }
-                need = sk_select<BLOCK>(p, ctl, t, my_rank);
-                SKT(ctl, 9);
-                if (need == 0xFFFFFFFFu) { if (tid == 0) ctl->fail = 3; GP_SYNC(); return; }
-            }
-            if (!ovf) break;
+        GP_SYNC();
+        SKT(ctl, 8);
+        if (uni(ctl->ovf)) {
             GP_SYNC();
-            if (tid == 0) { ctl->ovf = 0; GP_OVF_COUNT(p, kOvfTopk); }
-            P *= 2; need = 0;
-            if (P > 64u) { if (tid == 0) ctl->fail = 4; GP_SYNC(); return; }
+            if (tid == 0) { ctl->ovf = 0; GP_OVF_COUNT(p, kOvfTopk); ctl->tk_t = t_c; ctl->tk_dig = (u32)round | (last ? 0x100u : 0u); }
             GP_SYNC();
-        }
+            [[clang::musttail]] return phase_sk_topk_parts<BLOCK, TG>(lds0, row_lo, row_hi, seed, n_pu, n_log);
+        }
+        need = sk_select<BLOCK>(p, ctl, t, my_rank);
+        SKT(ctl, 9);
+        if (need == 0xFFFFFFFFu) { if (tid == 0) ctl->fail = 3; GP_SYNC(); return 0u; }
         if (t_c <= 1u || last) break;
         if (need == K) {
             const double tau_fx = __builtin_floor(__longlong_as_double((long long)uni(ctl->kth_bits)) * p.sk_rscale * (1.0 - 1.0 / 1048576.0));
@@ -932,16 +1009,90 @@
         }
         if (tid == 0) zstat(ctl, zSweep2, 1);
     }
-    const long long out0 = row * (long long)p.K;
-    if ((u32)tid < need) {
-        const Cand cd = t.sel[tid];
-        const int node = p.unit_info[(u32)cd.key & p.node_mask];
-        __builtin_nontemporal_store(seed, &p.out_row[out0 + my_rank]);
-        __builtin_nontemporal_store(node, &p.out_col[out0 + my_rank]);
-        __builtin_nontemporal_store(__longlong_as_double((long long)cd.bits), &p.out_val[out0 + my_rank]);
-    }
-    publish_filled(p, row, need);
-    if (tid == 0) zstat(ctl, zFilled, need);
+    sk_write_row(p, ctl, t, row, seed, need, my_rank);
+    return 0u;
+}
+
+template <int BLOCK, bool TG>
+__device__ GP_PHASE_NOINLINE u32 phase_sk_topk_parts(u32 lds0, u32 row_lo, u32 row_hi, int seed, u32 n_pu, u32 n_log)
+{
+    KP p = kparams();
+    lds0 = uni(lds0); row_lo = uni(row_lo); row_hi = uni(row_hi); seed = uni(seed); n_pu = uni(n_pu); n_log = uni(n_log);
+    const SkView w = sk_view<BLOCK>(p, lds0);
+    CtlS* ctl = w.ctl;
+    const SkTop t = sk_top(p, w, TG ? 0u : n_pu);
+    const long long row = (long long)(((u64)row_hi << 32) | row_lo);
+    const int tid = threadIdx.x;
+    const u32 K = (u32)p.K;
+    u32 t_c = uni(ctl->tk_t);
+    const u32 dig = uni(ctl->tk_dig);
+    bool last = (dig & 0x100u) != 0u;
+    u32 need = 0, my_rank = 0;
+    const bool cl = (uni(ctl->k_solo_ok) & 2u) != 0u;
+    const u32 list_base = (n_log + 3u) & ~3u;
+    const bool list_ok = cl && (u64)list_base + n_log <= (u64)uni(ctl->k_log_cap);
+    bool resumed = true;
+    for (int round = (int)(dig & 0xFFu); ; ++round) {
+        u32 part = 0, np = resumed ? 2u : 1u, P0 = cl ? 1u : np, n_list = 0;
+        bool done_any = false, listed = false;
+        resumed = false;
+        for (;;) {
+            const u32 n_run = done_any ? need : 0u;
+            Cand mine; mine.bits = 0; mine.key = kEmpty; mine.pad = 0;
+            if ((u32)tid < n_run) mine = t.sel[tid];
+            GP_SYNC();
+            for (u32 i = tid; i < t.CA; i += BLOCK) { t.akeys[i] = kEmpty; t.avals[i] = 0.0; }
+            if (tid < 64) ctl->bcnt[tid] = 0;
+            if (tid == 0) { ctl->n_sel = 0; ctl->n_tie = 0; ctl->tk_wide = 0; ctl->kth_bits = ~0ull; if (!listed) ctl->n_list = 0; }
+            GP_SYNC();
+            if (n_run != 0u) {
+                if (mine.key != kEmpty) { t.akeys[t.CA - 1u - (u32)tid] = mine.key; t.avals[t.CA - 1u - (u32)tid] = __longlong_as_double((long long)mine.bits); }
+                GP_SYNC();
+            }
+            const bool building = np > 1u && list_ok && !listed;
+            if (listed)        phase_sk_topk_part<BLOCK, TG, 2>(lds0, n_pu, list_base, list_base + n_list, t_c, np, part, 0u);
+            else if (building) phase_sk_topk_part<BLOCK, TG, 1>(lds0, n_pu, 0u, n_log, t_c, np, part, list_base);
+            else               phase_sk_topk_part<BLOCK, TG, 0>(lds0, n_pu, 0u, n_log, t_c, np, part, 0u);
+            GP_SYNC();
+            SKT(ctl, 8);
+            if (uni(ctl->ovf)) {
+                GP_SYNC();
+                if (tid == 0) { ctl->ovf = 0; GP_OVF_COUNT(p, kOvfTopk); }
+                if (cl) { part *= 2; np *= 2; }
+                else { np *= 2; P0 = np; part = 0; need = 0; done_any = false; }
+                if (np > 64u) { if (tid == 0) ctl->fail = 4; GP_SYNC(); return 0u; }
+                GP_SYNC();
+                continue;
+            }
+            if (building) {
+                n_list = uni(ctl->n_list); listed = true;
+                if (tid == 0) GP_OVF_ADD(p, kSkListed, n_list);
+            } else if (listed && tid == 0) GP_OVF_COUNT(p, kSkListWalks);
+            need = sk_select<BLOCK>(p, ctl, t, my_rank);
+            SKT(ctl, 9);
+            if (need == 0xFFFFFFFFu) { if (tid == 0) ctl->fail = 3; GP_SYNC(); return 0u; }
+            done_any = true;
+            while (np > P0 && (part & 1u)) { part >>= 1; np >>= 1; }
+            ++part;
+            if (np == P0 && part == P0) break;
+            if (cl && need == K) {
+                const double tau_fx = __builtin_floor(__longlong_as_double((long long)uni(ctl->kth_bits)) * p.sk_rscale * (1.0 - 1.0 / 1048576.0));
+                if (tau_fx > (double)t_c) t_c = (u32)tau_fx;
+            }
+        }
+        if (t_c <= 1u || last) break;
+        if (need == K) {
+            const double tau_fx = __builtin_floor(__longlong_as_double((long long)uni(ctl->kth_bits)) * p.sk_rscale * (1.0 - 1.0 / 1048576.0));
+            if (tau_fx >= (double)t_c) break;
+            t_c = tau_fx >= 1.0 ? (u32)tau_fx : 1u;
+            last = true;
+        } else {
+            t_c = round >= 2 ? 1u : max(1u, t_c >> 4);
+        }
+        if (tid == 0) zstat(ctl, zSweep2, 1);
+    }
+    sk_write_row(p, ctl, t, row, seed, need, my_rank);
+    return 0u;
 }
 
 template <int BLOCK>
@@ -956,8 +1107,8 @@
         for (u32 i = 4u * threadIdx.x; i < w.MR + w.MU; i += 4u * BLOCK) *(u4*)&w.R[i] = z;
         n = w.CX;
     }
-    if (what == 3u) {
-        for (u32 i = 4u * threadIdx.x; i < w.MU; i += 4u * BLOCK) *(u4*)&w.U[i] = z;
+    if (what == 3u || what == 4u) {
+        if (what == 3u) for (u32 i = 4u * threadIdx.x; i < w.MU; i += 4u * BLOCK) *(u4*)&w.U[i] = z;
         for (u32 i = threadIdx.x; i < n; i += BLOCK) w.xvals[at + i] = 0.0;
         return;
     }
@@ -991,7 +1142,7 @@
     }
     const u32 units = (seed_deg + (1u << kUnitShift) - 1u) >> kUnitShift;
     const u32 k_lc = uni(ctl->k_log_cap), k_so = uni(ctl->k_solo_ok), k_dm = uni(ctl->k_direct_max);
-    const bool merged = (p.solo & 2u) != 0u && k_so != 0u && pushes && room && L >= 2u && seed_deg <= kSkSoloEdges && seed_deg <= k_dm &&
+    const bool merged = (p.solo & 2u) != 0u && (k_so & 1u) != 0u && pushes && room && L >= 2u && seed_deg <= kSkSoloEdges && seed_deg <= k_dm &&
                         (u64)units <= p.bt_cap && (u64)1u + seed_deg <= (u64)k_lc && (u64)2u + kSkSoloEdges + 4u <= (u64)pu_cap;
     if (merged && wave_id() != 0u) return 1u;
     if (tid == 0) {
@@ -1023,6 +1174,8 @@
     return 1u;
 }
 
+template <int BLOCK>
+__device__ GP_PHASE_NOINLINE u32 phase_sk_level_redo(u32 lds0, u32 lvl, u32 L);
 template <int BLOCK, bool REDO = false>
 __device__ __forceinline__ u32 phase_sk_level(u32 lds0, u32 lvl, u32 L)
 {
@@ -1050,17 +1203,18 @@
     const u32 seg_base = log_pos;
     const u32 pu_next = pu_cur + n_ent_cur + (has_dang_cur ? 1u : 0u);
     const u32 cur = lvl & 1u;
-    if (tid == 0) {
+    if (!REDO && tid == 0) {
         nx->dangling = 0.0; nx->n_dangling = 0; nx->n_rec = 0; nx->alloc = 0ull; nx->pad1 = sk_io_pack(pu_next, log_pos + n_rec);
+        ctl->n_list = 0;
         ctl->tot_pu = pu_next; ctl->tot_log = log_pos + n_rec; ctl->max_e = max(ctl->max_e, e_cur);
         ctl->lv_has_dang = has_dang_cur ? 1u : 0u; ctl->lv_dang = dang_cur;
         if (has_dang_cur) w.arch[pu_cur + n_ent_cur] = uni(c_) * dang_cur;
-        if (!REDO) zstat(ctl, zLevels, 1);
+        zstat(ctl, zLevels, 1);
     }
     const double cs = uni(c_) * uni(krs_);
     const double cnext = last ? 0.0 : uni(c1_);
     SKT(ctl, 6);
-    if (last) {
+    if (!REDO && last) {
         phase_sk_stream<BLOCK, 2>(lds0, cur, n_ent_cur, e_cur, seg_base, cs, 0u, pu_cur, 1u, 0u);
         SKT(ctl, 3);
         return 0u;
@@ -1076,7 +1230,7 @@
         const u32 est = direct ? (n_rec > direct_max ? 2u * n_rec : 0u) : (u32)(((u64)n_rec * q) >> 10);
         while (P0 < 64u && est > P0 * capx) ++P0;
     }
-    const bool solo = !REDO && uni(kso_) && direct && e_cur <= kSkSoloEdges && n_ent_cur >= 1u && n_ent_cur <= 64u &&
+    const bool solo = !REDO && (uni(kso_) & 1u) != 0u && direct && e_cur <= kSkSoloEdges && n_ent_cur >= 1u && n_ent_cur <= 64u &&
                       (u64)pu_next + kSkSoloEdges + 4u <= pu_cap;
     if (REDO) {
     } else if (solo) {
@@ -1095,40 +1249,78 @@
         SKT(ctl, direct ? 1 : 2); SKT_COUNT(ctl, direct ? 13 : 14, 1);
     }
     const bool by_log = !direct;
-    bool u_dirty = !direct, first = true;
-    u32 part = 0, np = P0;
-    bool level_done = false;
-    if (solo) {
-        if (!uni(ctl->ovf)) level_done = true;
-        else { capx = CX; }
-    }
-    if (REDO) capx = CX;
-    if (!level_done)
-    for (;;) {
-        if (!(first && direct && P0 == 1u)) {
+    if (!REDO) {
+        if (by_log && P0 == 1u) {
             SKT2_BEGIN(ctl);
-            if (by_log) phase_sk_filter<BLOCK>(lds0, seg_base, n_rec, capx, pu_cur, np, part);
-            else        phase_sk_stream<BLOCK, 3>(lds0, cur, n_ent_cur, e_cur, seg_base, cs, capx, pu_cur, np, part);
+            phase_sk_filter<BLOCK, 0>(lds0, seg_base, n_rec, capx, pu_cur, 1u, 0u, 0u);
             SKT2(ctl, 2);
             GP_SYNC();
             SKT2(ctl, 3);
             SKT(ctl, 4); SKT_COUNT(ctl, 11, 1);
         }
+        if (P0 > 1u || uni(ctl->ovf)) return phase_sk_level_redo<BLOCK>(lds0, lvl, L);
+        if (solo) return uni(ctl->fail) ? 0u : 1u;
+        SKT2_BEGIN(ctl);
+        phase_sk_scan<BLOCK>(lds0, capx, lvl & 1u, cur ^ 1u, by_log ? 1u : 0u, by_log ? s_n : 0u, pu_next, cnext);
+        SKT2(ctl, 9);
+        GP_SYNC();
+        SKT2(ctl, 10);
+        SKT(ctl, 5); SKT_COUNT(ctl, 12, 1);
+        if (uni(ctl->fail)) return 0u;
+        if (tid == 0 && by_log) {
+            const u32 obs = min(2048u, (u32)(1280.0f * (float)nx->n_rec * __frcp_rn((float)n_rec)) + 8u);
+            const u32 old_q = ctl->cand_q[lvl];
+            ctl->cand_q[lvl] = max(obs, old_q - (old_q >> 3));
+        }
+        return 1u;
+    }
+    bool u_dirty = !direct, s_dirty = !direct;
+    bool first = uni(ctl->ovf) != 0u;
+    u32 part = 0, np = P0;
+    bool building = false;
+    const u32 list_base = (seg_base + n_rec + 3u) & ~3u;
+    const bool list_ok = by_log && (uni(kso_) & 2u) != 0u && (u64)list_base + n_rec <= (u64)uni(klc_);
+    bool listed = false;
+    u32 n_list = 0;
+    for (;;) {
+        if (!first) {
+            SKT2_BEGIN(ctl);
+            building = list_ok && !listed && np > 1u;
+            if (!by_log)       phase_sk_stream<BLOCK, 3>(lds0, cur, n_ent_cur, e_cur, seg_base, cs, capx, pu_cur, np, part);
+            else if (listed)   phase_sk_filter<BLOCK, 2>(lds0, list_base, n_list, capx, pu_cur, np, part, 0u);
+            else if (building) phase_sk_filter<BLOCK, 1>(lds0, seg_base, n_rec, capx, pu_cur, np, part, list_base);
+            else               phase_sk_filter<BLOCK, 0>(lds0, seg_base, n_rec, capx, pu_cur, np, part, 0u);
+            SKT2(ctl, 2);
+            GP_SYNC();
+            SKT2(ctl, 3);
+            SKT(ctl, 4); SKT_COUNT(ctl, 11, 1);
+        }
         first = false;
         if (uni(ctl->ovf)) {
             phase_sk_wipe<BLOCK>(lds0, 2u, by_log ? cap0 : CX, 0u);
             GP_SYNC();
-            if (tid == 0) { ctl->ovf = 0; GP_OVF_COUNT(p, kOvfLevel); }
+            if (tid == 0) { ctl->ovf = 0; ctl->n_list = 0; GP_OVF_COUNT(p, kOvfLevel); }
             if (!by_log) capx = CX;
             if (np < 0x10000u) { part *= 2; np *= 2; GP_SYNC(); continue; }
             if (tid == 0) ctl->fail = 5;
             GP_SYNC();
             break;
         }
-        const bool final_part = np == P0 && part + 1u == P0;
+        if (building) {
+            n_list = uni(ctl->n_list); listed = true;
+            if (tid == 0) GP_OVF_ADD(p, kSkListed, n_list);
+        } else if (listed && tid == 0) GP_OVF_COUNT(p, kSkListWalks);
+        bool final_part = np == P0 && part + 1u == P0;
+        if (listed) {
+            u32 pp = part, nn = np;
+            while (nn > P0 && (pp & 1u)) { pp >>= 1; nn >>= 1; }
+            final_part = nn == P0 && pp + 1u == P0;
+        }
+        const bool u_dead = u_dirty && (final_part || listed);
         SKT2_BEGIN(ctl);
-        phase_sk_scan<BLOCK>(lds0, capx, lvl & 1u, cur ^ 1u, final_part && u_dirty ? s_n : 0u, pu_next, cnext);
-        if (final_part) u_dirty = false;
+        phase_sk_scan<BLOCK>(lds0, capx, lvl & 1u, cur ^ 1u, u_dead ? 1u : 0u, final_part && s_dirty ? s_n : 0u, pu_next, cnext);
+        if (u_dead) u_dirty = false;
+        if (final_part) s_dirty = false;
         SKT2(ctl, 9);
         GP_SYNC();
         SKT2(ctl, 10);
@@ -1138,8 +1330,8 @@
         ++part;
         if (np == P0 && part == P0) break;
     }
-    if (u_dirty) {
-        phase_sk_wipe<BLOCK>(lds0, 3u, s_n, cap0);
+    if (s_dirty) {
+        phase_sk_wipe<BLOCK>(lds0, u_dirty ? 3u : 4u, s_n, cap0);
         GP_SYNC();
     }
     if (uni(ctl->fail)) return 0u;
@@ -1152,7 +1344,7 @@
 }
 
 template <int BLOCK>
-__device__ GP_PHASE_NOINLINE u32 phase_sk_level1_redo(u32 lds0, u32 L) { return phase_sk_level<BLOCK, true>(lds0, 1u, L); }
+__device__ GP_PHASE_NOINLINE u32 phase_sk_level_redo(u32 lds0, u32 lvl, u32 L) { return phase_sk_level<BLOCK, true>(lds0, lvl, L); }
 
 template <int BLOCK>
 __device__ __forceinline__ void gfpush_sk_rows()
@@ -1176,8 +1368,9 @@
         ctl->max_e = 0; ctl->max_log = 0;
         ctl->k_log_cap = (u32)min(p.log_cap, (u64)0xFFFFFFFFu); ctl->k_pu_cap = (u32)min((u64)kSkMaxPushers, p.arch_cap);
         ctl->k_direct_max = min(p.sk_direct_max, 3u * (w.CX / 4u)); ctl->k_cx = w.CX; ctl->k_rscale = p.sk_rscale;
-        ctl->k_solo_ok = (p.solo & 1u) && p.push_cap >= (u64)kSkSoloEdges + 4u &&
-                         (double)p.bt_cap >= (p.rmax > 0.0 ? fmin((double)p.nnz, 1.001 / p.rmax + 16.0) : (double)p.nnz) / (double)(1u << kUnitShift) + 4.0 ? 1u : 0u;
+        ctl->k_solo_ok = ((p.solo & 1u) && p.push_cap >= (u64)kSkSoloEdges + 4u &&
+                          (double)p.bt_cap >= (p.rmax > 0.0 ? fmin((double)p.nnz, 1.001 / p.rmax + 16.0) : (double)p.nnz) / (double)(1u << kUnitShift) + 4.0 ? 1u : 0u) |
+                         ((p.solo & 4u) ? 2u : 0u);
     }
     const long long n_rows = p.n_seeds;
     const u32 L = (u32)p.n_coef - 1u;
@@ -1207,7 +1400,7 @@
         SKT(ctl, 0); SKT_COUNT(ctl, 15, 1);
         if (lvl == 2u) {
             SKT_COUNT(ctl, 13, 1);
-            if (uni(ctl->ovf)) lvl = uni(phase_sk_level1_redo<BLOCK>(lds0, L)) ? 2u : L + 1u;
+            if (uni(ctl->ovf)) lvl = uni(phase_sk_level_redo<BLOCK>(lds0, 1u, L)) ? 2u : L + 1u;
         }
         for (; lvl <= L; ++lvl)
             if (!uni(phase_sk_level<BLOCK>(lds0, lvl, L))) break;
```
